# dbdexter-dev/meteor_demod

Measured on AMD Instinct MI355X. Metric: IQ Msamples/s demodulated (whole node), higher is better.
Workload: dtype f32

## Files before the change

meteor_demod_amd/csrc/demod_kernel_gat.hip:

```cpp
#include "rotwin_body.h"
#include "hip_host.h"

namespace {

typedef float gpair_t __attribute__((ext_vector_type(2)));
typedef float gquad_t __attribute__((ext_vector_type(4)));
typedef __attribute__((address_space(3))) const gquad_t lds_gquad;
typedef __attribute__((address_space(3))) const float lds_gfloat;

template <int FMT> struct GFmt;
template <> struct GFmt<16> {
	enum { G = 4 };
	__device__ static __forceinline__ gpair_t get(const uint4 &q, int k) { const uint32_t w = (&q.x)[k]; return gpair_t{ (float)(int)(int16_t)(w & 0xFFFFu), (float)((int)w >> 16) }; }
	__device__ static __forceinline__ gpair_t one(uint32_t w) { return gpair_t{ (float)(int)(int16_t)(w & 0xFFFFu), (float)((int)w >> 16) }; }
};
template <> struct GFmt<8> {
	enum { G = 8 };
	__device__ static __forceinline__ gpair_t get(const uint4 &q, int k) { const uint32_t w = (&q.x)[k >> 1] >> (16 * (k & 1)); return gpair_t{ (float)((int)(w & 0xFFu) - 128), (float)((int)((w >> 8) & 0xFFu) - 128) }; }
	__device__ static __forceinline__ gpair_t one(uint16_t w) { return gpair_t{ (float)((int)(w & 0xFFu) - 128), (float)((int)(w >> 8) - 128) }; }
};
template <> struct GFmt<32> {
	enum { G = 2 };
	__device__ static __forceinline__ gpair_t get(const uint4 &q, int k) { return gpair_t{ __uint_as_float((&q.x)[2 * k]), __uint_as_float((&q.x)[2 * k + 1]) }; }
	__device__ static __forceinline__ gpair_t one(float2 w) { return gpair_t{ w.x, w.y }; }
};

template <int KT, int FMT>
struct WinG {
	static constexpr int G = GFmt<FMT>::G, kTaps = KT, kBack = KT - 1, AMAX = G - 1, NS = KT + AMAX, NW = 4 * ((NS + 3) / 4), SLIDE = 4, MAXSL = 1, DEPTH = 1,
	                     BLOCK = MDEMOD_RW_BLOCK, ROTN = 1, RING = 32, REGSLOTS = 0;
	static constexpr bool GATHER = true;
	static_assert(NS % G == 0 && NS / G <= 36, "whole 16-byte loads, and few enough of them to stay in registers");
	typedef typename RFmt<FMT>::sample_t sample_t;
	__device__ __forceinline__ void setup(uint32_t) {}
	__device__ static __forceinline__ void put_history(const float2 *, bool, int) {}
	__device__ static __forceinline__ void put_init(const RGran<FMT> (&)[1], int) {}
	__device__ static __forceinline__ void put(const RGran<FMT> (&)[1], int) {}
	__device__ static __forceinline__ void fir(uint32_t, int, int, const DemodConsts &, int, float &, float &) {}

	__device__ static __forceinline__ void
	fir_gather(uint32_t ctab_addr, const sample_t *src, const float2 *hist, int v, int n, int bank, const DemodConsts &C, float &re, float &im)
	{
		const int oldest = v - kBack - (KT - 1);
		const int d = oldest & (G - 1);
		const int start = oldest - d;
		const int o = AMAX - d;
		const uint32_t row = ctab_addr + 4u * (uint32_t)(__mul24(bank * 4 + (o & 3), C.ctab_row_stride) + (o & ~3));
		gpair_t acc = { 0.0f, 0.0f };
		if (__builtin_expect(md_all(start >= 0 && start + NS <= n), 1)) {
			uint4 raw[NS / G];
#pragma unroll
			for (int g = 0; g < NS / G; g++) __builtin_memcpy(&raw[g], src + start + G * g, 16);
#pragma unroll
			for (int s4 = 0; s4 < NS / 4; s4++) {
				gquad_t c = { 0.0f, 0.0f, 0.0f, 0.0f };
				c = *(lds_gquad *)(row + 16u * (uint32_t)s4);
				const float cf[4] = { c.x, c.y, c.z, c.w };
#pragma unroll
				for (int k = 0; k < 4; k++) {
					const int slot = 4 * s4 + k;
					const gpair_t smp = GFmt<FMT>::get(raw[slot / G], slot % G);
					const gpair_t p = smp * cf[k];
					acc = acc + p;
				}
			}
			if constexpr (NS % 4 != 0) {
#pragma unroll
				for (int slot = NS / 4 * 4; slot < NS; slot++) {
					const float cf = *(lds_gfloat *)(row + 4u * (uint32_t)slot);
					const gpair_t p = GFmt<FMT>::get(raw[slot / G], slot % G) * cf;
					acc = acc + p;
				}
			}
		} else {
#pragma unroll 1
			for (int k = 0; k < KT; k++) {
				const int idx = oldest + k;
				gpair_t smp;
				if (idx < 0) { const float2 h = hist[kBack + idx]; smp.x = h.x; smp.y = h.y; }
				else smp = GFmt<FMT>::one(src[idx]);
				const float cf = *(lds_gfloat *)(row + 4u * (uint32_t)(d + k));
				const gpair_t p = smp * cf;
				acc = acc + p;
			}
		}
		re = acc.x; im = acc.y;
	}
};

template <int FMT, int OQPSK, int KT>
__global__ void __launch_bounds__(MDEMOD_RW_BLOCK, 2)
demod_kernel_gat(const DemodLaunch L)
{
	rotwin_demod<WinG<KT, FMT>, FMT, OQPSK, 0>(L);
}

template <int FMT, int OQPSK, int KT>
hipError_t
launch_gat(const DemodLaunch &L, size_t lds_bytes, hipStream_t stream)
{
	const uint32_t blocks = (L.n_streams + MDEMOD_RW_BLOCK - 1) / MDEMOD_RW_BLOCK;
	auto kfn = demod_kernel_gat<FMT, OQPSK, KT>;
	return mdm_launch(kfn, dim3(blocks), dim3(MDEMOD_RW_BLOCK), lds_bytes, stream, L);
}

}

template <int FMT>
static hipError_t
launch_gat_fmt(const DemodLaunch &L, int long_filter, size_t lds_bytes, hipStream_t stream)
{
	if constexpr (FMT != 32)
		if (long_filter) return L.c.oqpsk ? launch_gat<FMT, 1, 129>(L, lds_bytes, stream) : launch_gat<FMT, 0, 129>(L, lds_bytes, stream);
	if (long_filter) return hipErrorInvalidValue;
	return L.c.oqpsk ? launch_gat<FMT, 1, 65>(L, lds_bytes, stream) : launch_gat<FMT, 0, 65>(L, lds_bytes, stream);
}

hipError_t
mdemod_launch_demod_gat(const DemodLaunch &L, int fmt, int long_filter, size_t lds_bytes, hipStream_t stream)
{
	switch (fmt) {
	case 16: return launch_gat_fmt<16>(L, long_filter, lds_bytes, stream);
	case 8:  return launch_gat_fmt<8>(L, long_filter, lds_bytes, stream);
	case 32: return launch_gat_fmt<32>(L, long_filter, lds_bytes, stream);
	default: return hipErrorInvalidValue;
	}
}
```

meteor_demod_amd/csrc/demod_kernel_rot.hip:

```cpp
#include "rotwin_body.h"
#include "hip_host.h"
#ifdef ROTWIN_ASM_HEADER
#include ROTWIN_ASM_HEADER
#else
#include "rotwin_asm.h"
#endif

namespace {

static_assert(ROTWIN_NCH * 8 == 80, "window = ten chunks of eight");


__device__ __forceinline__ void
rot_fir(uint32_t row_addr, int rot, int flags, float &re, float &im)
{
	int tmp;
#if ROTWIN_PK == 1 || ROTWIN_PK == 3
	typedef float pair_t __attribute__((ext_vector_type(2)));
	pair_t acc = { 0.0f, 0.0f }, p0, p1;
	asm volatile(ROTWIN_FIR_ASM
	             : [acc] "+v"(acc), [p0] "=&v"(p0), [p1] "=&v"(p1), [tmp] "=&s"(tmp)
	             : [addr] "v"(row_addr), [rot] "s"(rot), [flags] "s"(flags)
	             : "vcc", "scc", ROTWIN_COEF_CLOBBERS);
	re = acc.x; im = acc.y;
#else
	float t0, t1, t2, t3;
	asm volatile(ROTWIN_FIR_ASM
	             : [ar] "=&v"(re), [ai] "=&v"(im), [t0] "=&v"(t0), [t1] "=&v"(t1), [t2] "=&v"(t2), [t3] "=&v"(t3), [tmp] "=&s"(tmp)
	             : [addr] "v"(row_addr), [rot] "s"(rot), [flags] "s"(flags)
	             : "vcc", "scc", ROTWIN_COEF_CLOBBERS);
#endif
}

template <int FMT> __device__ __forceinline__ void rot_put(const RGran<FMT> &a, const RGran<FMT> &b, int q);
template <> __device__ __forceinline__ void
rot_put<16>(const RGran<16> &a, const RGran<16> &b, int q)
{
	int tmp;
	asm volatile(ROTWIN_PUT_S16_ASM
	             : [tmp] "=&s"(tmp)
	             : [g0] "v"(a.w[0]), [g1] "v"(a.w[1]), [g2] "v"(a.w[2]), [g3] "v"(a.w[3]),
	               [g4] "v"(b.w[0]), [g5] "v"(b.w[1]), [g6] "v"(b.w[2]), [g7] "v"(b.w[3]), [rot] "s"(q)
	             : "vcc", "scc", "v255", "memory");
}
template <> __device__ __forceinline__ void
rot_put<8>(const RGran<8> &a, const RGran<8> &b, int q)
{
	const uint32_t g0 = a.w[0] ^ 0x80808080u, g1 = a.w[1] ^ 0x80808080u, g2 = b.w[0] ^ 0x80808080u, g3 = b.w[1] ^ 0x80808080u;
	int tmp;
	asm volatile(ROTWIN_PUT_U8_ASM
	             : [tmp] "=&s"(tmp)
	             : [g0] "v"(g0), [g1] "v"(g1), [g2] "v"(g2), [g3] "v"(g3), [rot] "s"(q)
	             : "vcc", "scc", "v255", "memory");
}
__device__ __forceinline__ void
rot_put_floats(const uint32_t (&f)[16], int q)
{
	int tmp;
	asm volatile(ROTWIN_PUT_F32_ASM
	             : [tmp] "=&s"(tmp)
	             : [f0] "v"(f[0]), [f1] "v"(f[1]), [f2] "v"(f[2]), [f3] "v"(f[3]), [f4] "v"(f[4]), [f5] "v"(f[5]), [f6] "v"(f[6]), [f7] "v"(f[7]),
	               [f8] "v"(f[8]), [f9] "v"(f[9]), [f10] "v"(f[10]), [f11] "v"(f[11]), [f12] "v"(f[12]), [f13] "v"(f[13]), [f14] "v"(f[14]), [f15] "v"(f[15]),
	               [rot] "s"(q)
	             : "vcc", "scc", "v255", "memory");
}
template <> __device__ __forceinline__ void
rot_put<32>(const RGran<32> &a, const RGran<32> &b, int q)
{
	uint32_t f[16];
#pragma unroll
	for (int i = 0; i < 8; i++) { f[i] = a.w[i]; f[8 + i] = b.w[i]; }
	rot_put_floats(f, q);
}

template <int FMT, int COMPACT = 0, int BLK = MDEMOD_RW_BLOCK>
struct WinF {
	static constexpr int kTaps = 65, kBack = 64, NW = 80, SLIDE = 8, AMAX = NW - kTaps, MAXSL = 1, DEPTH = 1, BLOCK = BLK, ROTN = NW / SLIDE, RING = 32;
	static constexpr bool GATHER = false;
	__device__ __forceinline__ void setup(uint32_t) {}
#ifndef ROT_REGSLOTS
#define ROT_REGSLOTS 0
#endif
	static constexpr int REGSLOTS = ROT_REGSLOTS;
	__device__ static __forceinline__ void put_history(const float2 *hist, bool valid, int q)
	{
		const uint4 *h4 = reinterpret_cast<const uint4 *>(hist);
		uint32_t f[16];
#pragma unroll
		for (int i = 0; i < 4; i++) {
			uint4 h = h4[i];
			if (!valid) h = make_uint4(0, 0, 0, 0);
			f[4 * i] = h.x; f[4 * i + 1] = h.y; f[4 * i + 2] = h.z; f[4 * i + 3] = h.w;
		}
		rot_put_floats(f, q);
	}
	__device__ static __forceinline__ void put(const RGran<FMT> (&g)[2], int q) { rot_put<FMT>(g[0], g[1], q); }
	__device__ static __forceinline__ void put_init(const RGran<FMT> (&g)[2], int q) { put(g, q); }
	__device__ static __forceinline__ void fir(uint32_t ctab_addr, int a, int bank, const DemodConsts &C, int rot, float &re, float &im)
	{
		const int o = AMAX - a;
		uint32_t row_addr;
		if (COMPACT) row_addr = rot_mad24((uint32_t)(bank * 4 + (o & 3)), 4u * (uint32_t)C.ctab_row_stride, ctab_addr + 4u * (uint32_t)(o & ~3));
		else row_addr = rot_mad24(rot_mad24((uint32_t)a, (uint32_t)C.interp, (uint32_t)bank), 4u * (uint32_t)C.ctab_row_stride, ctab_addr);
		static_assert(AMAX == 15, "two bits of a / 4");
		const int lo1 = md_all(a >= 8) ? 2 : 0, hi1 = md_all(a < 8) ? 1 : 3;
		const int q_lo = md_all(a >= 4 * (lo1 + 1)) ? lo1 + 1 : lo1, q_hi = md_all(a < 4 * hi1) ? hi1 - 1 : hi1;
		const int flags = ((1 << q_lo) - 1) | (((1 << (3 - q_hi)) - 1) << 3);
#ifdef ROT_EXP_NOSKIP
		int f0 = __builtin_amdgcn_readfirstlane(flags);
		asm volatile("s_and_b32 %0, %0, 0" : "+s"(f0) : : "scc");
		rot_fir(row_addr, rot, f0, re, im);
#else
		rot_fir(row_addr, rot, __builtin_amdgcn_readfirstlane(flags), re, im);
#endif
	}
};

typedef float pair_t2 __attribute__((ext_vector_type(2)));

template <int NA>
__device__ __forceinline__ void
rot_fir_acc(uint32_t addr, int rot, int last, pair_t2 &acc)
{
	int tmp;
	if constexpr (NA == 10)
		asm volatile(ROTWIN_FIR_ACC_ASM
		             : [acc] "+v"(acc), [tmp] "=&s"(tmp)
		             : [addr] "v"(addr), [rot] "s"(rot), [last] "s"(last)
		             : "vcc", "scc", ROTWIN_COEF_CLOBBERS, ROTWIN_ACC_CLOBBERS);
	else if constexpr (NA == 2)
		asm volatile(ROTWIN_FIR_ACC2_ASM
		             : [acc] "+v"(acc), [tmp] "=&s"(tmp)
		             : [addr] "v"(addr), [rot] "s"(rot), [last] "s"(last)
		             : "vcc", "scc", ROTWIN_COEF_CLOBBERS, ROTWIN_ACC_CLOBBERS);
	else
		asm volatile(ROTWIN_FIR_ACC5_ASM
		             : [acc] "+v"(acc), [tmp] "=&s"(tmp)
		             : [addr] "v"(addr), [rot] "s"(rot), [last] "s"(last)
		             : "vcc", "scc", ROTWIN_COEF_CLOBBERS, ROTWIN_ACC_CLOBBERS);
}
#define ROT_F16_OPERANDS \
	[f0] "v"(f[0]), [f1] "v"(f[1]), [f2] "v"(f[2]), [f3] "v"(f[3]), [f4] "v"(f[4]), [f5] "v"(f[5]), [f6] "v"(f[6]), [f7] "v"(f[7]), \
	[f8] "v"(f[8]), [f9] "v"(f[9]), [f10] "v"(f[10]), [f11] "v"(f[11]), [f12] "v"(f[12]), [f13] "v"(f[13]), [f14] "v"(f[14]), [f15] "v"(f[15])
template <int NA>
__device__ __forceinline__ void
rot_migrate(const uint32_t (&f)[16], int q)
{
	int tmp;
	if constexpr (NA == 10)
		asm volatile(ROTWIN_MIGRATE_ASM : [tmp] "=&s"(tmp) : ROT_F16_OPERANDS, [rot] "s"(q) : "vcc", "scc", "v255", ROTWIN_ACC_CLOBBERS, "memory");
	else if constexpr (NA == 2)
		asm volatile(ROTWIN_MIGRATE2_ASM : [tmp] "=&s"(tmp) : ROT_F16_OPERANDS, [rot] "s"(q) : "vcc", "scc", "v255", ROTWIN_ACC_CLOBBERS, "memory");
	else
		asm volatile(ROTWIN_MIGRATE5_ASM : [tmp] "=&s"(tmp) : ROT_F16_OPERANDS, [rot] "s"(q) : "vcc", "scc", "v255", ROTWIN_ACC_CLOBBERS, "memory");
}
template <int NA>
__device__ __forceinline__ void
rot_put_acc(const uint32_t (&f)[16], int q)
{
	int tmp;
	if constexpr (NA == 10)
		asm volatile(ROTWIN_PUT_ACC_ASM : [tmp] "=&s"(tmp) : ROT_F16_OPERANDS, [rot] "s"(q) : "vcc", "scc", ROTWIN_ACC_CLOBBERS, "memory");
	else if constexpr (NA == 2)
		asm volatile(ROTWIN_PUT_ACC2_ASM : [tmp] "=&s"(tmp) : ROT_F16_OPERANDS, [rot] "s"(q) : "vcc", "scc", ROTWIN_ACC_CLOBBERS, "memory");
	else
		asm volatile(ROTWIN_PUT_ACC5_ASM : [tmp] "=&s"(tmp) : ROT_F16_OPERANDS, [rot] "s"(q) : "vcc", "scc", ROTWIN_ACC_CLOBBERS, "memory");
}

template <int BLK, int NA, int MSL>
struct WinH {
	static constexpr int NR = 10, SLIDE = 8, NW = SLIDE * (NR + NA), kTaps = NA == 10 ? 129 : 65, kBack = kTaps - 1, AMAX = NW - kTaps, MAXSL = MSL, DEPTH = MSL,
	                     BLOCK = BLK, ROTN = NR, RING = 32, REGSLOTS = 0;
	static constexpr bool GATHER = false;
	static_assert((NA == 10 || NA == 2 || NA == 5) && AMAX == (NA == 5 ? 55 : 31) && kBack % SLIDE == 0, "wide (160 slots, 129 taps), mid (96 slots, 65 taps) or far (120 slots, 65 taps)");
	__device__ __forceinline__ void setup(uint32_t) {}
	__device__ static __forceinline__ void place(const uint32_t (&f)[16], int c)
	{
		if (c < NR) rot_put_floats(f, c);
		else rot_put_acc<NA>(f, c - NR);
	}
	__device__ static __forceinline__ void put_history(const float2 *hist, bool valid, int c)
	{
		const uint4 *h4 = reinterpret_cast<const uint4 *>(hist);
		uint32_t f[16];
#pragma unroll
		for (int i = 0; i < 4; i++) {
			uint4 h = h4[i];
			if (!valid) h = make_uint4(0, 0, 0, 0);
			f[4 * i] = h.x; f[4 * i + 1] = h.y; f[4 * i + 2] = h.z; f[4 * i + 3] = h.w;
		}
		place(f, c);
	}
	__device__ static __forceinline__ void put_init(const RGran<32> (&g)[2], int c)
	{
		uint32_t f[16];
#pragma unroll
		for (int i = 0; i < 8; i++) { f[i] = g[0].w[i]; f[8 + i] = g[1].w[i]; }
		place(f, c);
	}
	__device__ static __forceinline__ void put(const RGran<32> (&g)[2], int q)
	{
		uint32_t f[16];
#pragma unroll
		for (int i = 0; i < 8; i++) { f[i] = g[0].w[i]; f[8 + i] = g[1].w[i]; }
		rot_migrate<NA>(f, q);
	}
	__device__ static __forceinline__ void fir(uint32_t ctab_addr, int a, int bank, const DemodConsts &C, int rot, float &re, float &im)
	{
		const int o = AMAX - a;
		const uint32_t row = ctab_addr + 4u * (uint32_t)(__mul24(bank * 4 + (o & 3), C.ctab_row_stride) + (o & ~3));
		const int flags = (md_all(a >= 8) ? 3 : 0) | ((NA != 10 && md_all(a <= 7)) ? 16 : 0);
		rot_fir(row, rot, __builtin_amdgcn_readfirstlane(flags), re, im);
		if (NA == 10 || md_any(a >= 16)) {
			int last;
			if (NA == 10) last = 6 + (md_any(a >= 8) ? 1 : 0) + (md_any(a >= 16) ? 1 : 0) + (md_any(a >= 24) ? 1 : 0);
			else {
				last = md_any(a >= 24) ? 1 : 0;
				if (NA == 5) last += (md_any(a >= 32) ? 1 : 0) + (md_any(a >= 40) ? 1 : 0) + (md_any(a >= 48) ? 1 : 0);
			}
			pair_t2 acc = { re, im };
			rot_fir_acc<NA>(row + 4u * 80u, NA == 10 ? rot : (NA == 2 ? (rot & 1) : (rot >= 5 ? rot - 5 : rot)), __builtin_amdgcn_readfirstlane(last), acc);
			re = acc.x; im = acc.y;
		}
	}
};

template <int OQPSK, int BLK, int NA, int MSL>
__global__ void __launch_bounds__(BLK, 1) __attribute__((amdgpu_num_vgpr(ROTWIN_LIMIT)))
demod_kernel_roth(const DemodLaunch L)
{
	rotwin_demod<WinH<BLK, NA, MSL>, 32, OQPSK, 0>(L);
}

template <int FMT, int OQPSK, int KS, int COMPACT, int LUT>
__global__ void __launch_bounds__(LUT ? MDEMOD_RW_LUT_BLOCK : MDEMOD_RW_BLOCK, 2) __attribute__((amdgpu_num_vgpr(ROTWIN_LIMIT / 2)))
demod_kernel_rot(const DemodLaunch L)
{
	rotwin_demod<WinF<FMT, COMPACT, LUT ? MDEMOD_RW_LUT_BLOCK : MDEMOD_RW_BLOCK>, FMT, OQPSK, KS, LUT>(L);
}

template <int FMT, int OQPSK, int KS, int COMPACT = 0, int LUT = 0>
hipError_t
launch_rot_ks(const DemodLaunch &L, size_t lds_bytes, hipStream_t stream)
{
	constexpr int BLOCK = LUT ? MDEMOD_RW_LUT_BLOCK : MDEMOD_RW_BLOCK;
	const uint32_t blocks = (L.n_streams + BLOCK - 1) / BLOCK;
	auto kfn = demod_kernel_rot<FMT, OQPSK, KS, COMPACT, LUT>;
	return mdm_launch(kfn, dim3(blocks), dim3(BLOCK), lds_bytes, stream, L);
}

template <int FMT, int OQPSK>
hipError_t
launch_rot(const DemodLaunch &L, int compact, size_t lds_bytes, hipStream_t stream)
{
	constexpr int KS = OQPSK ? 6 : 14;
	if (compact) return launch_rot_ks<FMT, OQPSK, 0, 1>(L, lds_bytes, stream);
	return L.c.sin_lut && L.c.step_safe == KS && L.c.clock_tab ? launch_rot_ks<FMT, OQPSK, KS, 0, 1>(L, lds_bytes, stream) : launch_rot_ks<FMT, OQPSK, 0>(L, lds_bytes, stream);
}

}

template <int OQPSK, int BLK, int NA, int MSL>
static hipError_t
launch_roth(const DemodLaunch &L, size_t lds_bytes, hipStream_t stream)
{
	const uint32_t blocks = (L.n_streams + BLK - 1) / BLK;
	auto kfn = demod_kernel_roth<OQPSK, BLK, NA, MSL>;
	return mdm_launch(kfn, dim3(blocks), dim3(BLK), lds_bytes, stream, L);
}

hipError_t
mdemod_launch_demod_roth(const DemodLaunch &L, int geom, int many_slides, size_t lds_bytes, hipStream_t stream)
{
	if (geom == 1 && many_slides) return L.c.oqpsk ? launch_roth<1, 256, 2, 3>(L, lds_bytes, stream) : launch_roth<0, 256, 2, 3>(L, lds_bytes, stream);
	if (geom == 1) return L.c.oqpsk ? launch_roth<1, 256, 2, 2>(L, lds_bytes, stream) : launch_roth<0, 256, 2, 2>(L, lds_bytes, stream);
	if (geom == 2) return L.c.oqpsk ? launch_roth<1, 256, 5, 3>(L, lds_bytes, stream) : launch_roth<0, 256, 5, 3>(L, lds_bytes, stream);
	return L.c.oqpsk ? launch_roth<1, 256, 10, 2>(L, lds_bytes, stream) : launch_roth<0, 256, 10, 2>(L, lds_bytes, stream);
}

hipError_t
mdemod_launch_demod_rot(const DemodLaunch &L, int fmt, int compact, size_t lds_bytes, hipStream_t stream)
{
	switch (fmt) {
	case 16: return L.c.oqpsk ? launch_rot<16, 1>(L, compact, lds_bytes, stream) : launch_rot<16, 0>(L, compact, lds_bytes, stream);
	case 8:  return L.c.oqpsk ? launch_rot<8, 1>(L, compact, lds_bytes, stream) : launch_rot<8, 0>(L, compact, lds_bytes, stream);
	case 32: return L.c.oqpsk ? launch_rot<32, 1>(L, compact, lds_bytes, stream) : launch_rot<32, 0>(L, compact, lds_bytes, stream);
	default: return hipErrorInvalidValue;
	}
}
```

meteor_demod_amd/csrc/demod_kernel_rotp.hip:

```cpp
#include "rotwin_body.h"
#include "hip_host.h"
#ifdef ROTPK_ASM_HEADER
#include ROTPK_ASM_HEADER
#else
#include "rotpk_asm.h"
#endif

namespace {

typedef float pair_t __attribute__((ext_vector_type(2)));

template <int GEO> struct GeoP;
#ifndef ROTP_WIDE_DEPTH
#define ROTP_WIDE_DEPTH 1
#endif
#ifndef ROTP_MID_DEPTH
#define ROTP_MID_DEPTH 1
#endif
#ifndef ROTP_FAR_DEPTH
#define ROTP_FAR_DEPTH 2
#endif
template <> struct GeoP<0> { static constexpr int kTaps = 129, NW = MDEMOD_RW_WIDE_NW, MAXSL = 1, DEPTH = ROTP_WIDE_DEPTH, BLOCK = MDEMOD_RW_WIDE_BLOCK; };
template <> struct GeoP<1> { static constexpr int kTaps = 65, NW = MDEMOD_RW_MID_NW, MAXSL = 1, DEPTH = ROTP_MID_DEPTH, BLOCK = MDEMOD_RW_BLOCK; };
#ifndef ROTP_FAR_MAXSL
#define ROTP_FAR_MAXSL 2
#endif
template <> struct GeoP<2> { static constexpr int kTaps = 65, NW = MDEMOD_RW_FAR_NW, MAXSL = ROTP_FAR_MAXSL, DEPTH = ROTP_FAR_DEPTH, BLOCK = MDEMOD_RW_BLOCK; };
static_assert(MDEMOD_RW_WIDE_NW == 160 && MDEMOD_RW_MID_NW == 96 && MDEMOD_RW_FAR_NW == 112, "gen_rotpk_asm.py: GEOS");

template <int GEO, int FMT> struct AsmP;
#if ROTPK_FORM == 0
#define ROTP_FIR_CALL(TEXT, CLOB)                                                                                             \
	float ar = 0.0f, ai = 0.0f;                                                                                               \
	asm volatile(TEXT : [ar] "+v"(ar), [ai] "+v"(ai), [addr] "+v"(addr), [cnt] "+s"(cnt), [tmp] "=&s"(tmp)                    \
	             : [entry] "s"(entry), [sub] "s"(sub) : "vcc", "scc", CLOB);                                                \
	re = ar; im = ai;
#else
#define ROTP_FIR_CALL(TEXT, CLOB)                                                                                             \
	pair_t acc = { 0.0f, 0.0f };                                                                                              \
	asm volatile(TEXT : [acc] "+v"(acc), [addr] "+v"(addr), [cnt] "+s"(cnt), [tmp] "=&s"(tmp)                                 \
	             : [entry] "s"(entry), [sub] "s"(sub) : "vcc", "scc", CLOB);                                                \
	re = acc.x; im = acc.y;
#endif
#define ROTP_ASM(GEO, NAME, FMT)                                                                                              \
	template <> struct AsmP<GEO, FMT> {                                                                                       \
		__device__ static __forceinline__ void fir(uint32_t addr, int entry, int sub, int cnt, float &re, float &im)          \
		{                                                                                                                     \
			int tmp;                                                                                                          \
			ROTP_FIR_CALL(ROTPK_##NAME##_##FMT##_FIR_ASM, ROTPK_##NAME##_##FMT##_CLOBBERS)                                     \
		}                                                                                                                     \
		__device__ static __forceinline__ void put(const uint32_t (&g)[FMT == 16 ? 16 : 8], int q);                           \
	};
ROTP_ASM(0, WIDE, 16) ROTP_ASM(0, WIDE, 8) ROTP_ASM(1, MID, 16) ROTP_ASM(1, MID, 8) ROTP_ASM(2, FAR, 16) ROTP_ASM(2, FAR, 8)

#define ROTP_PUT16(GEO, NAME)                                                                                                 \
	__device__ __forceinline__ void AsmP<GEO, 16>::put(const uint32_t (&g)[16], int q)                                        \
	{                                                                                                                         \
		int tmp;                                                                                                              \
		asm volatile(ROTPK_##NAME##_16_PUT_ASM                                                                                \
		             : [tmp] "=&s"(tmp)                                                                                       \
		             : [g0] "v"(g[0]), [g1] "v"(g[1]), [g2] "v"(g[2]), [g3] "v"(g[3]), [g4] "v"(g[4]), [g5] "v"(g[5]), [g6] "v"(g[6]),  \
		               [g7] "v"(g[7]), [g8] "v"(g[8]), [g9] "v"(g[9]), [g10] "v"(g[10]), [g11] "v"(g[11]), [g12] "v"(g[12]),  \
		               [g13] "v"(g[13]), [g14] "v"(g[14]), [g15] "v"(g[15]), [rot] "s"(q)                                     \
		             : "vcc", "scc", "v255", "memory");                                                                       \
	}
#define ROTP_PUT8(GEO, NAME)                                                                                                  \
	__device__ __forceinline__ void AsmP<GEO, 8>::put(const uint32_t (&g)[8], int q)                                          \
	{                                                                                                                         \
		int tmp;                                                                                                              \
		asm volatile(ROTPK_##NAME##_8_PUT_ASM                                                                                 \
		             : [tmp] "=&s"(tmp)                                                                                       \
		             : [g0] "v"(g[0]), [g1] "v"(g[1]), [g2] "v"(g[2]), [g3] "v"(g[3]), [g4] "v"(g[4]), [g5] "v"(g[5]), [g6] "v"(g[6]),  \
		               [g7] "v"(g[7]), [rot] "s"(q)                                                                           \
		             : "vcc", "scc", "v255", "memory");                                                                       \
	}
ROTP_PUT16(0, WIDE) ROTP_PUT16(1, MID) ROTP_PUT16(2, FAR) ROTP_PUT8(0, WIDE) ROTP_PUT8(1, MID) ROTP_PUT8(2, FAR)

template <int GEO, int FMT>
struct WinP {
	static constexpr int kTaps = GeoP<GEO>::kTaps, kBack = kTaps - 1, NW = GeoP<GEO>::NW, SLIDE = 16, AMAX = NW - kTaps,
	                     MAXSL = GeoP<GEO>::MAXSL, DEPTH = GeoP<GEO>::DEPTH, BLOCK = GeoP<GEO>::BLOCK, NCH = NW / SLIDE, GD = FMT == 16 ? 16 : 8, REGSLOTS = 0, ROTN = NCH, RING = 32;
	static constexpr bool GATHER = false;
	__device__ __forceinline__ void setup(uint32_t) {}
	static_assert(kBack % SLIDE == 0 && NW % SLIDE == 0, "history and window are whole chunks");

	__device__ static __forceinline__ void put_history(const float2 *hist, bool valid, int q)
	{
		uint32_t g[GD];
#pragma unroll
		for (int k = 0; k < 16; k++) {
			float2 h = hist[k];
			if (!valid) h = make_float2(0.0f, 0.0f);
			if (FMT == 16) {
				g[k] = ((uint32_t)(int)h.x & 0xFFFFu) | ((uint32_t)(int)h.y << 16);
			} else {
				const uint32_t s = (uint32_t)(((int)h.x + 128) & 0xFF) | ((uint32_t)(((int)h.y + 128) & 0xFF) << 8);
				if (k & 1) g[k / 2] |= s << 16; else g[k / 2] = s;
			}
		}
		AsmP<GEO, FMT>::put(g, q);
	}
	__device__ static __forceinline__ void put(const RGran<FMT> (&gr)[4], int q)
	{
		uint32_t g[GD];
#pragma unroll
		for (int i = 0; i < 4; i++)
#pragma unroll
			for (int j = 0; j < GD / 4; j++) g[i * (GD / 4) + j] = gr[i].w[j];
		AsmP<GEO, FMT>::put(g, q);
	}
	__device__ static __forceinline__ void put_init(const RGran<FMT> (&gr)[4], int q) { put(gr, q); }
	__device__ static __forceinline__ void fir(uint32_t ctab_addr, int a, int bank, const DemodConsts &C, int rot, float &re, float &im)
	{
		const int o = AMAX - a;
		uint32_t addr = rot_mad24((uint32_t)(bank * 4 + (o & 3)), 4u * (uint32_t)C.ctab_row_stride, ctab_addr + 4u * (uint32_t)(o & ~3));
		constexpr int QB = AMAX / 4 >= 8 ? 4 : 3;
		static_assert(AMAX / 4 < (1 << QB) && (kTaps - 1) % 4 == 0, "alignments in groups of four");
		int q_lo = 0, q_hi = (1 << QB) - 1;
#pragma unroll
		for (int b = QB - 1; b >= 0; b--) {
			const int t = q_lo + (1 << b);
			q_lo = md_all(a >= 4 * t) ? t : q_lo;
			const int u = q_hi - (1 << b);
			q_hi = md_all(a < 4 * (u + 1)) ? u : q_hi;
		}
		q_lo = __builtin_amdgcn_readfirstlane(q_lo); q_hi = __builtin_amdgcn_readfirstlane(q_hi);
		const int c_lo = q_lo >> 2;
		int chunk = rot + c_lo;
		chunk = chunk >= NCH ? chunk - NCH : chunk;
		const int sub = q_lo & 3;
		constexpr int XS = ROTPK_EXIT / 4;
		const int cnt = (q_hi + (kTaps - 1) / 4) / XS - q_lo / XS;
		AsmP<GEO, FMT>::fir(addr + 64u * (uint32_t)c_lo, __builtin_amdgcn_readfirstlane(chunk), __builtin_amdgcn_readfirstlane(sub), __builtin_amdgcn_readfirstlane(cnt), re, im);
	}
};

#define ROTP_KERNEL(GEO, NAME, FMT, OQ)                                                                                       \
	__global__ void __launch_bounds__(GeoP<GEO>::BLOCK, 2) __attribute__((amdgpu_num_vgpr(ROTPK_##NAME##_##FMT##_LIMIT / 2)))  \
	demod_kernel_rotp_##NAME##_##FMT##_##OQ(const DemodLaunch L) { rotwin_demod<WinP<GEO, FMT>, FMT, OQ, 0>(L); }
__global__ void __launch_bounds__(GeoP<0>::BLOCK, 2) __attribute__((amdgpu_num_vgpr(ROTPK_WIDE_16_LIMIT / 2)))
demod_kernel_rotp_WIDE_16_0_ks109(const DemodLaunch L) { rotwin_demod<WinP<0, 16>, 16, 0, 109, 1>(L); }
ROTP_KERNEL(0, WIDE, 16, 0) ROTP_KERNEL(0, WIDE, 16, 1) ROTP_KERNEL(0, WIDE, 8, 0) ROTP_KERNEL(0, WIDE, 8, 1)
ROTP_KERNEL(1, MID, 16, 0) ROTP_KERNEL(1, MID, 16, 1) ROTP_KERNEL(1, MID, 8, 0) ROTP_KERNEL(1, MID, 8, 1)
ROTP_KERNEL(2, FAR, 16, 0) ROTP_KERNEL(2, FAR, 16, 1) ROTP_KERNEL(2, FAR, 8, 0) ROTP_KERNEL(2, FAR, 8, 1)

typedef void (*rotp_kernel_t)(const DemodLaunch);

hipError_t
launch_rotp(rotp_kernel_t kfn, int block, const DemodLaunch &L, size_t lds_bytes, hipStream_t stream)
{
	const uint32_t blocks = (L.n_streams + block - 1) / block;
	return mdm_launch(kfn, dim3(blocks), dim3(block), lds_bytes, stream, L);
}

}

hipError_t
mdemod_launch_demod_rotp(const DemodLaunch &L, int fmt, int geom , size_t lds_bytes, hipStream_t stream)
{
	if ((fmt != 16 && fmt != 8) || geom < 0 || geom > 2) return hipErrorInvalidValue;
	static const rotp_kernel_t table[3][2][2] = {
		{ { demod_kernel_rotp_WIDE_16_0, demod_kernel_rotp_WIDE_16_1 }, { demod_kernel_rotp_WIDE_8_0, demod_kernel_rotp_WIDE_8_1 } },
		{ { demod_kernel_rotp_MID_16_0, demod_kernel_rotp_MID_16_1 }, { demod_kernel_rotp_MID_8_0, demod_kernel_rotp_MID_8_1 } },
		{ { demod_kernel_rotp_FAR_16_0, demod_kernel_rotp_FAR_16_1 }, { demod_kernel_rotp_FAR_8_0, demod_kernel_rotp_FAR_8_1 } },
	};
	static const int blocks[3] = { GeoP<0>::BLOCK, GeoP<1>::BLOCK, GeoP<2>::BLOCK };
	if (geom == 0 && fmt == 16 && !L.c.oqpsk && L.c.step_safe == 109 && L.c.sin_lut) return launch_rotp(demod_kernel_rotp_WIDE_16_0_ks109, blocks[0], L, lds_bytes, stream);
	return launch_rotp(table[geom][fmt == 16 ? 0 : 1][L.c.oqpsk ? 1 : 0], blocks[geom], L, lds_bytes, stream);
}
```

meteor_demod_amd/csrc/gen_rotwin_asm.py:

```python
#!/usr/bin/env python3
import os
import sys

WB = 96
CB = None
NCH = 10
PAIRWAIT = int(os.environ.get("ROTWIN_PAIRWAIT", "1"))
DC = int(os.environ.get("ROTWIN_DC", "1"))
NBUF = 2 * (DC + 1) if PAIRWAIT else 4
CB = 96 - 4 * NBUF
PK = int(os.environ.get("ROTWIN_PK", "1"))
TB = CB - 4
CHB = 32


def q(lines):
    return "\n".join('\t"%s\\n\\t"' % l for l in lines)


def jump(tag, n):
    return [
        "s_getpc_b64 vcc",
        ".L%s_pc_%%=:" % tag,
        "s_mul_i32 %%[tmp], %%[rot], (.L%s_1_%%= - .L%s_0_%%=)" % (tag, tag),
        "s_add_u32 %%[tmp], %%[tmp], (.L%s_0_%%= - .L%s_pc_%%=)" % (tag, tag),
        "s_add_u32 vcc_lo, vcc_lo, %[tmp]",
        "s_addc_u32 vcc_hi, vcc_hi, 0",
        "s_setpc_b64 vcc",
    ]


def fir():
    NH, D = 2 * NCH, 3
    def load(h):
        b = CB + 4 * (h % NBUF)
        return "ds_read_b128 v[%d:%d], %%[addr] offset:%d" % (b, b + 3, 16 * h)
    L = []
    if PK in (0, 2):
        L += ["v_mov_b32 %[ar], 0", "v_mov_b32 %[ai], 0"]
    L += [load(h) for h in range(2 * DC if PAIRWAIT else D)]
    L += jump("fir", NCH)
    for r in range(NCH):
        L += [".Lfir_%d_%%=:" % r]
        for h in range(NH):
            c = h // 2
            if PAIRWAIT:
                if h % 2 == 0:
                    L += [load(x) for x in (h + 2 * DC, h + 2 * DC + 1) if x < NH]
                    L += ["s_waitcnt lgkmcnt(%d)" % min(2 * DC, max(0, NH - 2 - h))]
            else:
                if h + D < NH:
                    L += [load(h + D)]
                L += ["s_waitcnt lgkmcnt(%d)" % min(D, NH - 1 - h)]
            if h < 3:
                L += ["s_bitcmp1_b32 %%[flags], %d" % h, "s_cbranch_scc1 .Lfir_%d_s%d_%%=" % (r, h)]
            if h >= NH - 3:
                L += ["s_bitcmp1_b32 %%[flags], %d" % (3 + NH - 1 - h), "s_cbranch_scc1 .Lfir_%d_s9_%%=" % r]
            hb = CB + 4 * (h % NBUF)
            wq = WB + 16 * ((c + r) % NCH) + 8 * (h & 1)
            if PK == 1:
                def mul(j):
                    return ["v_pk_mul_f32 %%[p%d], v[%d:%d], v[%d:%d] op_sel:[0,%d] op_sel_hi:[1,%d]"
                            % (j & 1, wq + 2 * j, wq + 2 * j + 1, hb + 2 * (j // 2), hb + 2 * (j // 2) + 1, j & 1, j & 1)]
                def add(j):
                    return ["v_pk_add_f32 %%[acc], %%[acc], %%[p%d]" % (j & 1)]
            elif PK == 2:
                def mul(j):
                    t = TB + 2 * (j & 1)
                    return ["v_pk_mul_f32 v[%d:%d], v[%d:%d], v[%d:%d] op_sel:[0,%d] op_sel_hi:[1,%d]"
                            % (t, t + 1, wq + 2 * j, wq + 2 * j + 1, hb + 2 * (j // 2), hb + 2 * (j // 2) + 1, j & 1, j & 1)]
                def add(j):
                    t = TB + 2 * (j & 1)
                    return ["v_add_f32 %%[ar], %%[ar], v%d" % t, "v_add_f32 %%[ai], %%[ai], v%d" % (t + 1)]
            elif PK == 3:
                def mul(j):
                    t = TB + 2 * (j & 1)
                    return ["v_mul_f32 v%d, v%d, v%d" % (t, hb + j, wq + 2 * j), "v_mul_f32 v%d, v%d, v%d" % (t + 1, hb + j, wq + 2 * j + 1)]
                def add(j):
                    t = TB + 2 * (j & 1)
                    return ["v_pk_add_f32 %%[acc], %%[acc], v[%d:%d]" % (t, t + 1)]
            else:
                def mul(j):
                    t = "%%[t%d]" % (2 * (j & 1)), "%%[t%d]" % (2 * (j & 1) + 1)
                    return ["v_mul_f32 %s, v%d, v%d" % (t[0], hb + j, wq + 2 * j),
                            "v_mul_f32 %s, v%d, v%d" % (t[1], hb + j, wq + 2 * j + 1)]
                def add(j):
                    t = "%%[t%d]" % (2 * (j & 1)), "%%[t%d]" % (2 * (j & 1) + 1)
                    return ["v_add_f32 %%[ar], %%[ar], %s" % t[0], "v_add_f32 %%[ai], %%[ai], %s" % t[1]]
            L += mul(0)
            for j in range(4):
                if j + 1 < 4:
                    L += mul(j + 1)
                L += add(j)
            if h < 3:
                L += [".Lfir_%d_s%d_%%=:" % (r, h)]
        L += [".Lfir_%d_s9_%%=:" % r, "s_branch .Lfir_end_%="]
    L += [".Lfir_end_%=:", "s_waitcnt lgkmcnt(0)"]
    return L


def put(kind):
    L = ["s_nop 1"] if kind == "u8" else []
    L += jump("put", NCH)
    for r in range(NCH):
        L += [".Lput_%d_%%=:" % r]
        wq = WB + 16 * r
        for s in range(8):
            for comp in range(2):
                dst = wq + 2 * s + comp
                if kind == "s16":
                    L += ["v_cvt_f32_i32_sdwa v%d, sext(%%[g%d]) dst_sel:DWORD dst_unused:UNUSED_PAD src0_sel:WORD_%d" % (dst, s, comp)]
                elif kind == "u8":
                    L += ["v_cvt_f32_i32_sdwa v%d, sext(%%[g%d]) dst_sel:DWORD dst_unused:UNUSED_PAD src0_sel:BYTE_%d" % (dst, s // 2, 2 * (s & 1) + comp)]
                else:
                    L += ["v_mov_b32 v%d, %%[f%d]" % (dst, 2 * s + comp)]
        L += ["s_branch .Lput_end_%="]
    L += [".Lput_end_%=:"]
    return L


AB = 96


def fir_acc(NA, tag):
    NH = 2 * NA
    lo = 6 if NA == NCH else 0
    def load(h):
        b = CB + 4 * (h % 3)
        return "ds_read_b128 v[%d:%d], %%[addr] offset:%d" % (b, b + 3, 16 * h)
    L = [load(h) for h in range(2)]
    L += jump(tag, NA)
    for r in range(NA):
        L += [".L%s_%d_%%=:" % (tag, r)]
        for h in range(NH):
            c = h // 2
            if h + 2 < NH:
                L += [load(h + 2)]
            L += ["s_waitcnt lgkmcnt(%d)" % min(2, NH - 1 - h)]
            hb = CB + 4 * (h % 3)
            aq = AB + 16 * ((c + r) % NA) + 8 * (h & 1)
            def rd(j):
                t = CB + 12 + 2 * (j & 1)
                return ["v_accvgpr_read_b32 v%d, a%d" % (t, aq + 2 * j), "v_accvgpr_read_b32 v%d, a%d" % (t + 1, aq + 2 * j + 1)]
            def mul(j):
                t = CB + 12 + 2 * (j & 1)
                return ["v_pk_mul_f32 v[%d:%d], v[%d:%d], v[%d:%d] op_sel:[0,%d] op_sel_hi:[1,%d]" % (t, t + 1, t, t + 1, hb + 2 * (j // 2), hb + 2 * (j // 2) + 1, j & 1, j & 1)]
            def add(j):
                t = CB + 12 + 2 * (j & 1)
                return ["v_pk_add_f32 %%[acc], %%[acc], v[%d:%d]" % (t, t + 1)]
            L += rd(0) + rd(1) + mul(0) + mul(1) + add(0) + rd(2) + add(1) + rd(3) + mul(2) + mul(3) + add(2) + add(3)
            if h % 2 == 1 and lo <= c < NA - 1:
                L += ["s_cmp_eq_u32 %%[last], %d" % c, "s_cbranch_scc1 .L%s_end_%%=" % tag]
        L += ["s_branch .L%s_end_%%=" % tag]
    L += [".L%s_end_%%=:" % tag, "s_waitcnt lgkmcnt(0)"]
    return L


def migrate(NA, tag):
    assert NCH % NA == 0
    L = jump(tag, NCH)
    for r in range(NCH):
        L += [".L%s_%d_%%=:" % (tag, r)]
        L += ["v_accvgpr_read_b32 v%d, a%d" % (WB + 16 * r + k, AB + 16 * (r % NA) + k) for k in range(16)]
        L += ["v_accvgpr_write_b32 a%d, %%[f%d]" % (AB + 16 * (r % NA) + k, k) for k in range(16)]
        L += ["s_branch .L%s_end_%%=" % tag]
    L += [".L%s_end_%%=:" % tag]
    return L


def put_acc(NA, tag):
    L = jump(tag, NA)
    for r in range(NA):
        L += [".L%s_%d_%%=:" % (tag, r)]
        L += ["v_accvgpr_write_b32 a%d, %%[f%d]" % (AB + 16 * r + k, k) for k in range(16)]
        L += ["s_branch .L%s_end_%%=" % tag]
    L += [".L%s_end_%%=:" % tag]
    return L


def main():
    out = []
    out.append("/* GENERATED by gen_rotwin_asm.py - do not edit.  gfx950 assembly of the rotating register window. */")
    out.append("#ifndef MDEMOD_ROTWIN_ASM_H")
    out.append("#define MDEMOD_ROTWIN_ASM_H")
    out.append("#define ROTWIN_WB %d" % WB)
    out.append("#define ROTWIN_CB %d" % CB)
    out.append("#define ROTWIN_LIMIT %d   /* first register the compiler may not use */" % (TB if PK in (2, 3) else CB))
    out.append("#define ROTWIN_NCH %d" % NCH)
    out.append("#define ROTWIN_AB %d   /* first AccVGPR of the hybrid window's newer half */" % AB)
    out.append("#define ROTWIN_PK %d" % PK)
    out.append("#define ROTWIN_FIR_ASM \\\n" + q(fir()).replace("\n", " \\\n"))
    for kind in ("s16", "u8", "f32"):
        out.append("#define ROTWIN_PUT_%s_ASM \\\n" % kind.upper() + q(put(kind)).replace("\n", " \\\n"))
    for NA, sfx in ((NCH, ""), (2, "2"), (5, "5")):
        out.append("#define ROTWIN_FIR_ACC%s_ASM \\\n" % sfx + q(fir_acc(NA, "fira" + sfx)).replace("\n", " \\\n"))
        out.append("#define ROTWIN_MIGRATE%s_ASM \\\n" % sfx + q(migrate(NA, "mig" + sfx)).replace("\n", " \\\n"))
        out.append("#define ROTWIN_PUT_ACC%s_ASM \\\n" % sfx + q(put_acc(NA, "puta" + sfx)).replace("\n", " \\\n"))
    out.append("#define ROTWIN_ACC_CLOBBERS " + ", ".join('"a%d"' % i for i in range(AB, AB + 16 * NCH)))
    out.append("#define ROTWIN_COEF_CLOBBERS " + ", ".join('"v%d"' % i for i in range(TB if PK in (2, 3) else CB, WB)))
    out.append("#endif")
    sys.stdout.write("\n".join(out) + "\n")


if __name__ == "__main__":
    main()
```

meteor_demod_amd/csrc/rotwin_asm.h:

```cpp
#ifndef MDEMOD_ROTWIN_ASM_H
#define MDEMOD_ROTWIN_ASM_H
#define ROTWIN_WB 96
#define ROTWIN_CB 80
#define ROTWIN_LIMIT 80
#define ROTWIN_NCH 10
#define ROTWIN_AB 96
#define ROTWIN_PK 1
#define ROTWIN_FIR_ASM \
	"ds_read_b128 v[80:83], %[addr] offset:0\n\t" \
	"ds_read_b128 v[84:87], %[addr] offset:16\n\t" \
	"s_getpc_b64 vcc\n\t" \
	".Lfir_pc_%=:\n\t" \
	"s_mul_i32 %[tmp], %[rot], (.Lfir_1_%= - .Lfir_0_%=)\n\t" \
	"s_add_u32 %[tmp], %[tmp], (.Lfir_0_%= - .Lfir_pc_%=)\n\t" \
	"s_add_u32 vcc_lo, vcc_lo, %[tmp]\n\t" \
	"s_addc_u32 vcc_hi, vcc_hi, 0\n\t" \
	"s_setpc_b64 vcc\n\t" \
	".Lfir_0_%=:\n\t" \
	"ds_read_b128 v[88:91], %[addr] offset:32\n\t" \
	"ds_read_b128 v[92:95], %[addr] offset:48\n\t" \
	"s_waitcnt lgkmcnt(2)\n\t" \
	"s_bitcmp1_b32 %[flags], 0\n\t" \
	"s_cbranch_scc1 .Lfir_0_s0_%=\n\t" \
	"v_pk_mul_f32 %[p0], v[96:97], v[80:81] op_sel:[0,0] op_sel_hi:[1,0]\n\t" \
	"v_pk_mul_f32 %[p1], v[98:99], v[80:81] op_sel:[0,1] op_sel_hi:[1,1]\n\t" \
	"v_pk_add_f32 %[acc], %[acc], %[p0]\n\t" \
	"v_pk_mul_f32 %[p0], v[100:101], v[82:83] op_sel:[0,0] op_sel_hi:[1,0]\n\t" \
	"v_pk_add_f32 %[acc], %[acc], %[p1]\n\t" \
	"v_pk_mul_f32 %[p1], v[102:103], v[82:83] op_sel:[0,1] op_sel_hi:[1,1]\n\t" \
	"v_pk_add_f32 %[acc], %[acc], %[p0]\n\t" \
	"v_pk_add_f32 %[acc], %[acc], %[p1]\n\t" \
	".Lfir_0_s0_%=:\n\t" \
	"s_bitcmp1_b32 %[flags], 1\n\t" \
	"s_cbranch_scc1 .Lfir_0_s1_%=\n\t" \
	"v_pk_mul_f32 %[p0], v[104:105], v[84:85] op_sel:[0,0] op_sel_hi:[1,0]\n\t" \
	"v_pk_mul_f32 %[p1], v[106:107], v[84:85] op_sel:[0,1] op_sel_hi:[1,1]\n\t" \
	"v_pk_add_f32 %[acc], %[acc], %[p0]\n\t" \
	"v_pk_mul_f32 %[p0], v[108:109], v[86:87] op_sel:[0,0] op_sel_hi:[1,0]\n\t" \
	"v_pk_add_f32 %[acc], %[acc], %[p1]\n\t" \
	"v_pk_mul_f32 %[p1], v[110:111], v[86:87] op_sel:[0,1] op_sel_hi:[1,1]\n\t" \
	"v_pk_add_f32 %[acc], %[acc], %[p0]\n\t" \
	"v_pk_add_f32 %[acc], %[acc], %[p1]\n\t" \
	".Lfir_0_s1_%=:\n\t" \
	"ds_read_b128 v[80:83], %[addr] offset:64\n\t" \
	"ds_read_b128 v[84:87], %[addr] offset:80\n\t" \
	"s_waitcnt lgkmcnt(2)\n\t" \
	"s_bitcmp1_b32 %[flags], 2\n\t" \
	"s_cbranch_scc1 .Lfir_0_s2_%=\n\t" \
	"v_pk_mul_f32 %[p0], v[112:113], v[88:89] op_sel:[0,0] op_sel_hi:[1,0]\n\t" \
	"v_pk_mul_f32 %[p1], v[114:115], v[88:89] op_sel:[0,1] op_sel_hi:[1,1]\n\t" \
	"v_pk_add_f32 %[acc], %[acc], %[p0]\n\t" \
	"v_pk_mul_f32 %[p0], v[116:117], v[90:91] op_sel:[0,0] op_sel_hi:[1,0]\n\t" \
	"v_pk_add_f32 %[acc], %[acc], %[p1]\n\t" \
	"v_pk_mul_f32 %[p1], v[118:119], v[90:91] op_sel:[0,1] op_sel_hi:[1,1]\n\t" \
	"v_pk_add_f32 %[acc], %[acc], %[p0]\n\t" \
	"v_pk_add_f32 %[acc], %[acc], %[p1]\n\t" \
	".Lfir_0_s2_%=:\n\t" \
	"v_pk_mul_f32 %[p0], v[120:121], v[92:93] op_sel:[0,0] op_sel_hi:[1,0]\n\t" \
	"v_pk_mul_f32 %[p1], v[122:123], v[92:93] op_sel:[0,1] op_sel_hi:[1,1]\n\t" \
	"v_pk_add_f32 %[acc], %[acc], %[p0]\n\t" \
	"v_pk_mul_f32 %[p0], v[124:125], v[94:95] op_sel:[0,0] op_sel_hi:[1,0]\n\t" \
	"v_pk_add_f32 %[acc], %[acc], %[p1]\n\t" \
	"v_pk_mul_f32 %[p1], v[126:127], v[94:95] op_sel:[0,1] op_sel_hi:[1,1]\n\t" \
	"v_pk_add_f32 %[acc], %[acc], %[p0]\n\t" \
	"v_pk_add_f32 %[acc], %[acc], %[p1]\n\t" \
	"ds_read_b128 v[88:91], %[addr] offset:96\n\t" \
	"ds_read_b128 v[92:95], %[addr] offset:112\n\t" \
	"s_waitcnt lgkmcnt(2)\n\t" \
	"v_pk_mul_f32 %[p0], v[128:129], v[80:81] op_sel:[0,0] op_sel_hi:[1,0]\n\t" \
	"v_pk_mul_f32 %[p1], v[130:131], v[80:81] op_sel:[0,1] op_sel_hi:[1,1]\n\t" \
	"v_pk_add_f32 %[acc], %[acc], %[p0]\n\t" \
	"v_pk_mul_f32 %[p0], v[132:133], v[82:83] op_sel:[0,0] op_sel_hi:[1,0]\n\t" \
	"v_pk_add_f32 %[acc], %[acc], %[p1]\n\t" \
	"v_pk_mul_f32 %[p1], v[134:135], v[82:83] op_sel:[0,1] op_sel_hi:[1,1]\n\t" \
	"v_pk_add_f32 %[acc], %[acc], %[p0]\n\t" \
	"v_pk_add_f32 %[acc], %[acc], %[p1]\n\t" \
	"v_pk_mul_f32 %[p0], v[136:137], v[84:85] op_sel:[0,0] op_sel_hi:[1,0]\n\t" \
	"v_pk_mul_f32 %[p1], v[138:139], v[84:85] op_sel:[0,1] op_sel_hi:[1,1]\n\t" \
	"v_pk_add_f32 %[acc], %[acc], %[p0]\n\t" \
	"v_pk_mul_f32 %[p0], v[140:141], v[86:87] op_sel:[0,0] op_sel_hi:[1,0]\n\t" \
	"v_pk_add_f32 %[acc], %[acc], %[p1]\n\t" \
	"v_pk_mul_f32 %[p1], v[142:143], v[86:87] op_sel:[0,1] op_sel_hi:[1,1]\n\t" \
	"v_pk_add_f32 %[acc], %[acc], %[p0]\n\t" \
	"v_pk_add_f32 %[acc], %[acc], %[p1]\n\t" \
	"ds_read_b128 v[80:83], %[addr] offset:128\n\t" \
	"ds_read_b128 v[84:87], %[addr] offset:144\n\t" \
	"s_waitcnt lgkmcnt(2)\n\t" \
	"v_pk_mul_f32 %[p0], v[144:145], v[88:89] op_sel:[0,0] op_sel_hi:[1,0]\n\t" \
	"v_pk_mul_f32 %[p1], v[146:147], v[88:89] op_sel:[0,1] op_sel_hi:[1,1]\n\t" \
	"v_pk_add_f32 %[acc], %[acc], %[p0]\n\t" \
	"v_pk_mul_f32 %[p0], v[148:149], v[90:91] op_sel:[0,0] op_sel_hi:[1,0]\n\t" \
	"v_pk_add_f32 %[acc], %[acc], %[p1]\n\t" \
	"v_pk_mul_f32 %[p1], v[150:151], v[90:91] op_sel:[0,1] op_sel_hi:[1,1]\n\t" \
	"v_pk_add_f32 %[acc], %[acc], %[p0]\n\t" \
	"v_pk_add_f32 %[acc], %[acc], %[p1]\n\t" \
	"v_pk_mul_f32 %[p0], v[152:153], v[92:93] op_sel:[0,0] op_sel_hi:[1,0]\n\t" \
	"v_pk_mul_f32 %[p1], v[154:155], v[92:93] op_sel:[0,1] op_sel_hi:[1,1]\n\t" \
	"v_pk_add_f32 %[acc], %[acc], %[p0]\n\t" \
	"v_pk_mul_f32 %[p0], v[156:157], v[94:95] op_sel:[0,0] op_sel_hi:[1,0]\n\t" \
	"v_pk_add_f32 %[acc], %[acc], %[p1]\n\t" \
	"v_pk_mul_f32 %[p1], v[158:159], v[94:95] op_sel:[0,1] op_sel_hi:[1,1]\n\t" \
	"v_pk_add_f32 %[acc], %[acc], %[p0]\n\t" \
	"v_pk_add_f32 %[acc], %[acc], %[p1]\n\t" \
	"ds_read_b128 v[88:91], %[addr] offset:160\n\t" \
	"ds_read_b128 v[92:95], %[addr] offset:176\n\t" \
	"s_waitcnt lgkmcnt(2)\n\t" \
	"v_pk_mul_f32 %[p0], v[160:161], v[80:81] op_sel:[0,0] op_sel_hi:[1,0]\n\t" \
	"v_pk_mul_f32 %[p1], v[162:163], v[80:81] op_sel:[0,1] op_sel_hi:[1,1]\n\t" \
	"v_pk_add_f32 %[acc], %[acc], %[p0]\n\t" \
	"v_pk_mul_f32 %[p0], v[164:165], v[82:83] op_sel:[0,0] op_sel_hi:[1,0]\n\t" \
	"v_pk_add_f32 %[acc], %[acc], %[p1]\n\t" \
	"v_pk_mul_f32 %[p1], v[166:167], v[82:83] op_sel:[0,1] op_sel_hi:[1,1]\n\t" \
	"v_pk_add_f32 %[acc], %[acc], %[p0]\n\t" \
	"v_pk_add_f32 %[acc], %[acc], %[p1]\n\t" \
	"v_pk_mul_f32 %[p0], v[168:169], v[84:85] op_sel:[0,0] op_sel_hi:[1,0]\n\t" \
	"v_pk_mul_f32 %[p1], v[170:171], v[84:85] op_sel:[0,1] op_sel_hi:[1,1]\n\t" \
	"v_pk_add_f32 %[acc], %[acc], %[p0]\n\t" \
	"v_pk_mul_f32 %[p0], v[172:173], v[86:87] op_sel:[0,0] op_sel_hi:[1,0]\n\t" \
	"v_pk_add_f32 %[acc], %[acc], %[p1]\n\t" \
	"v_pk_mul_f32 %[p1], v[174:175], v[86:87] op_sel:[0,1] op_sel_hi:[1,1]\n\t" \
	"v_pk_add_f32 %[acc], %[acc], %[p0]\n\t" \
	"v_pk_add_f32 %[acc], %[acc], %[p1]\n\t" \
	"ds_read_b128 v[80:83], %[addr] offset:192\n\t" \
	"ds_read_b128 v[84:87], %[addr] offset:208\n\t" \
	"s_waitcnt lgkmcnt(2)\n\t" \
	"v_pk_mul_f32 %[p0], v[176:177], v[88:89] op_sel:[0,0] op_sel_hi:[1,0]\n\t" \
	"v_pk_mul_f32 %[p1], v[178:179], v[88:89] op_sel:[0,1] op_sel_hi:[1,1]\n\t" \
	"v_pk_add_f32 %[acc], %[acc], %[p0]\n\t" \
	"v_pk_mul_f32 %[p0], v[180:181], v[90:91] op_sel:[0,0] op_sel_hi:[1,0]\n\t" \
	"v_pk_add_f32 %[acc], %[acc], %[p1]\n\t" \
	"v_pk_mul_f32 %[p1], v[182:183], v[90:91] op_sel:[0,1] op_sel_hi:[1,1]\n\t" \
	"v_pk_add_f32 %[acc], %[acc], %[p0]\n\t" \
	"v_pk_add_f32 %[acc], %[acc], %[p1]\n\t" \
	"v_pk_mul_f32 %[p0], v[184:185], v[92:93] op_sel:[0,0] op_sel_hi:[1,0]\n\t" \
	"v_pk_mul_f32 %[p1], v[186:187], v[92:93] op_sel:[0,1] op_sel_hi:[1,1]\n\t" \
	"v_pk_add_f32 %[acc], %[acc], %[p0]\n\t" \
	"v_pk_mul_f32 %[p0], v[188:189], v[94:95] op_sel:[0,0] op_sel_hi:[1,0]\n\t" \
	"v_pk_add_f32 %[acc], %[acc], %[p1]\n\t" \
	"v_pk_mul_f32 %[p1], v[190:191], v[94:95] op_sel:[0,1] op_sel_hi:[1,1]\n\t" \
	"v_pk_add_f32 %[acc], %[acc], %[p0]\n\t" \
	"v_pk_add_f32 %[acc], %[acc], %[p1]\n\t" \
	"ds_read_b128 v[88:91], %[addr] offset:224\n\t" \
	"ds_read_b128 v[92:95], %[addr] offset:240\n\t" \
	"s_waitcnt lgkmcnt(2)\n\t" \
	"v_pk_mul_f32 %[p0], v[192:193], v[80:81] op_sel:[0,0] op_sel_hi:[1,0]\n\t" \
	"v_pk_mul_f32 %[p1], v[194:195], v[80:81] op_sel:[0,1] op_sel_hi:[1,1]\n\t" \
	"v_pk_add_f32 %[acc], %[acc], %[p0]\n\t" \
	"v_pk_mul_f32 %[p0], v[196:197], v[82:83] op_sel:[0,0] op_sel_hi:[1,0]\n\t" \
	"v_pk_add_f32 %[acc], %[acc], %[p1]\n\t" \
	"v_pk_mul_f32 %[p1], v[198:199], v[82:83] op_sel:[0,1] op_sel_hi:[1,1]\n\t" \
	"v_pk_add_f32 %[acc], %[acc], %[p0]\n\t" \
	"v_pk_add_f32 %[acc], %[acc], %[p1]\n\t" \
	"v_pk_mul_f32 %[p0], v[200:201], v[84:85] op_sel:[0,0] op_sel_hi:[1,0]\n\t" \
	"v_pk_mul_f32 %[p1], v[202:203], v[84:85] op_sel:[0,1] op_sel_hi:[1,1]\n\t" \
	"v_pk_add_f32 %[acc], %[acc], %[p0]\n\t" \
	"v_pk_mul_f32 %[p0], v[204:205], v[86:87] op_sel:[0,0] op_sel_hi:[1,0]\n\t" \
	"v_pk_add_f32 %[acc], %[acc], %[p1]\n\t" \
	"v_pk_mul_f32 %[p1], v[206:207], v[86:87] op_sel:[0,1] op_sel_hi:[1,1]\n\t" \
	"v_pk_add_f32 %[acc], %[acc], %[p0]\n\t" \
	"v_pk_add_f32 %[acc], %[acc], %[p1]\n\t" \
	"ds_read_b128 v[80:83], %[addr] offset:256\n\t" \
// ... 1953 lines not shown
	"v_cvt_f32_i32_sdwa v120, sext(%[g4]) dst_sel:DWORD dst_unused:UNUSED_PAD src0_sel:WORD_0\n\t" \
	"v_cvt_f32_i32_sdwa v121, sext(%[g4]) dst_sel:DWORD dst_unused:UNUSED_PAD src0_sel:WORD_1\n\t" \
	"v_cvt_f32_i32_sdwa v122, sext(%[g5]) dst_sel:DWORD dst_unused:UNUSED_PAD src0_sel:WORD_0\n\t" \
	"v_cvt_f32_i32_sdwa v123, sext(%[g5]) dst_sel:DWORD dst_unused:UNUSED_PAD src0_sel:WORD_1\n\t" \
	"v_cvt_f32_i32_sdwa v124, sext(%[g6]) dst_sel:DWORD dst_unused:UNUSED_PAD src0_sel:WORD_0\n\t" \
	"v_cvt_f32_i32_sdwa v125, sext(%[g6]) dst_sel:DWORD dst_unused:UNUSED_PAD src0_sel:WORD_1\n\t" \
	"v_cvt_f32_i32_sdwa v126, sext(%[g7]) dst_sel:DWORD dst_unused:UNUSED_PAD src0_sel:WORD_0\n\t" \
	"v_cvt_f32_i32_sdwa v127, sext(%[g7]) dst_sel:DWORD dst_unused:UNUSED_PAD src0_sel:WORD_1\n\t" \
	"s_branch .Lput_end_%=\n\t" \
	".Lput_2_%=:\n\t" \
	"v_cvt_f32_i32_sdwa v128, sext(%[g0]) dst_sel:DWORD dst_unused:UNUSED_PAD src0_sel:WORD_0\n\t" \
	"v_cvt_f32_i32_sdwa v129, sext(%[g0]) dst_sel:DWORD dst_unused:UNUSED_PAD src0_sel:WORD_1\n\t" \
	"v_cvt_f32_i32_sdwa v130, sext(%[g1]) dst_sel:DWORD dst_unused:UNUSED_PAD src0_sel:WORD_0\n\t" \
	"v_cvt_f32_i32_sdwa v131, sext(%[g1]) dst_sel:DWORD dst_unused:UNUSED_PAD src0_sel:WORD_1\n\t" \
	"v_cvt_f32_i32_sdwa v132, sext(%[g2]) dst_sel:DWORD dst_unused:UNUSED_PAD src0_sel:WORD_0\n\t" \
	"v_cvt_f32_i32_sdwa v133, sext(%[g2]) dst_sel:DWORD dst_unused:UNUSED_PAD src0_sel:WORD_1\n\t" \
	"v_cvt_f32_i32_sdwa v134, sext(%[g3]) dst_sel:DWORD dst_unused:UNUSED_PAD src0_sel:WORD_0\n\t" \
	"v_cvt_f32_i32_sdwa v135, sext(%[g3]) dst_sel:DWORD dst_unused:UNUSED_PAD src0_sel:WORD_1\n\t" \
	"v_cvt_f32_i32_sdwa v136, sext(%[g4]) dst_sel:DWORD dst_unused:UNUSED_PAD src0_sel:WORD_0\n\t" \
	"v_cvt_f32_i32_sdwa v137, sext(%[g4]) dst_sel:DWORD dst_unused:UNUSED_PAD src0_sel:WORD_1\n\t" \
	"v_cvt_f32_i32_sdwa v138, sext(%[g5]) dst_sel:DWORD dst_unused:UNUSED_PAD src0_sel:WORD_0\n\t" \
	"v_cvt_f32_i32_sdwa v139, sext(%[g5]) dst_sel:DWORD dst_unused:UNUSED_PAD src0_sel:WORD_1\n\t" \
	"v_cvt_f32_i32_sdwa v140, sext(%[g6]) dst_sel:DWORD dst_unused:UNUSED_PAD src0_sel:WORD_0\n\t" \
	"v_cvt_f32_i32_sdwa v141, sext(%[g6]) dst_sel:DWORD dst_unused:UNUSED_PAD src0_sel:WORD_1\n\t" \
	"v_cvt_f32_i32_sdwa v142, sext(%[g7]) dst_sel:DWORD dst_unused:UNUSED_PAD src0_sel:WORD_0\n\t" \
	"v_cvt_f32_i32_sdwa v143, sext(%[g7]) dst_sel:DWORD dst_unused:UNUSED_PAD src0_sel:WORD_1\n\t" \
	"s_branch .Lput_end_%=\n\t" \
	".Lput_3_%=:\n\t" \
	"v_cvt_f32_i32_sdwa v144, sext(%[g0]) dst_sel:DWORD dst_unused:UNUSED_PAD src0_sel:WORD_0\n\t" \
	"v_cvt_f32_i32_sdwa v145, sext(%[g0]) dst_sel:DWORD dst_unused:UNUSED_PAD src0_sel:WORD_1\n\t" \
	"v_cvt_f32_i32_sdwa v146, sext(%[g1]) dst_sel:DWORD dst_unused:UNUSED_PAD src0_sel:WORD_0\n\t" \
	"v_cvt_f32_i32_sdwa v147, sext(%[g1]) dst_sel:DWORD dst_unused:UNUSED_PAD src0_sel:WORD_1\n\t" \
	"v_cvt_f32_i32_sdwa v148, sext(%[g2]) dst_sel:DWORD dst_unused:UNUSED_PAD src0_sel:WORD_0\n\t" \
	"v_cvt_f32_i32_sdwa v149, sext(%[g2]) dst_sel:DWORD dst_unused:UNUSED_PAD src0_sel:WORD_1\n\t" \
	"v_cvt_f32_i32_sdwa v150, sext(%[g3]) dst_sel:DWORD dst_unused:UNUSED_PAD src0_sel:WORD_0\n\t" \
	"v_cvt_f32_i32_sdwa v151, sext(%[g3]) dst_sel:DWORD dst_unused:UNUSED_PAD src0_sel:WORD_1\n\t" \
	"v_cvt_f32_i32_sdwa v152, sext(%[g4]) dst_sel:DWORD dst_unused:UNUSED_PAD src0_sel:WORD_0\n\t" \
	"v_cvt_f32_i32_sdwa v153, sext(%[g4]) dst_sel:DWORD dst_unused:UNUSED_PAD src0_sel:WORD_1\n\t" \
	"v_cvt_f32_i32_sdwa v154, sext(%[g5]) dst_sel:DWORD dst_unused:UNUSED_PAD src0_sel:WORD_0\n\t" \
	"v_cvt_f32_i32_sdwa v155, sext(%[g5]) dst_sel:DWORD dst_unused:UNUSED_PAD src0_sel:WORD_1\n\t" \
	"v_cvt_f32_i32_sdwa v156, sext(%[g6]) dst_sel:DWORD dst_unused:UNUSED_PAD src0_sel:WORD_0\n\t" \
	"v_cvt_f32_i32_sdwa v157, sext(%[g6]) dst_sel:DWORD dst_unused:UNUSED_PAD src0_sel:WORD_1\n\t" \
	"v_cvt_f32_i32_sdwa v158, sext(%[g7]) dst_sel:DWORD dst_unused:UNUSED_PAD src0_sel:WORD_0\n\t" \
	"v_cvt_f32_i32_sdwa v159, sext(%[g7]) dst_sel:DWORD dst_unused:UNUSED_PAD src0_sel:WORD_1\n\t" \
	"s_branch .Lput_end_%=\n\t" \
	".Lput_4_%=:\n\t" \
	"v_cvt_f32_i32_sdwa v160, sext(%[g0]) dst_sel:DWORD dst_unused:UNUSED_PAD src0_sel:WORD_0\n\t" \
	"v_cvt_f32_i32_sdwa v161, sext(%[g0]) dst_sel:DWORD dst_unused:UNUSED_PAD src0_sel:WORD_1\n\t" \
	"v_cvt_f32_i32_sdwa v162, sext(%[g1]) dst_sel:DWORD dst_unused:UNUSED_PAD src0_sel:WORD_0\n\t" \
	"v_cvt_f32_i32_sdwa v163, sext(%[g1]) dst_sel:DWORD dst_unused:UNUSED_PAD src0_sel:WORD_1\n\t" \
	"v_cvt_f32_i32_sdwa v164, sext(%[g2]) dst_sel:DWORD dst_unused:UNUSED_PAD src0_sel:WORD_0\n\t" \
	"v_cvt_f32_i32_sdwa v165, sext(%[g2]) dst_sel:DWORD dst_unused:UNUSED_PAD src0_sel:WORD_1\n\t" \
	"v_cvt_f32_i32_sdwa v166, sext(%[g3]) dst_sel:DWORD dst_unused:UNUSED_PAD src0_sel:WORD_0\n\t" \
	"v_cvt_f32_i32_sdwa v167, sext(%[g3]) dst_sel:DWORD dst_unused:UNUSED_PAD src0_sel:WORD_1\n\t" \
	"v_cvt_f32_i32_sdwa v168, sext(%[g4]) dst_sel:DWORD dst_unused:UNUSED_PAD src0_sel:WORD_0\n\t" \
	"v_cvt_f32_i32_sdwa v169, sext(%[g4]) dst_sel:DWORD dst_unused:UNUSED_PAD src0_sel:WORD_1\n\t" \
	"v_cvt_f32_i32_sdwa v170, sext(%[g5]) dst_sel:DWORD dst_unused:UNUSED_PAD src0_sel:WORD_0\n\t" \
	"v_cvt_f32_i32_sdwa v171, sext(%[g5]) dst_sel:DWORD dst_unused:UNUSED_PAD src0_sel:WORD_1\n\t" \
	"v_cvt_f32_i32_sdwa v172, sext(%[g6]) dst_sel:DWORD dst_unused:UNUSED_PAD src0_sel:WORD_0\n\t" \
	"v_cvt_f32_i32_sdwa v173, sext(%[g6]) dst_sel:DWORD dst_unused:UNUSED_PAD src0_sel:WORD_1\n\t" \
	"v_cvt_f32_i32_sdwa v174, sext(%[g7]) dst_sel:DWORD dst_unused:UNUSED_PAD src0_sel:WORD_0\n\t" \
	"v_cvt_f32_i32_sdwa v175, sext(%[g7]) dst_sel:DWORD dst_unused:UNUSED_PAD src0_sel:WORD_1\n\t" \
	"s_branch .Lput_end_%=\n\t" \
	".Lput_5_%=:\n\t" \
	"v_cvt_f32_i32_sdwa v176, sext(%[g0]) dst_sel:DWORD dst_unused:UNUSED_PAD src0_sel:WORD_0\n\t" \
	"v_cvt_f32_i32_sdwa v177, sext(%[g0]) dst_sel:DWORD dst_unused:UNUSED_PAD src0_sel:WORD_1\n\t" \
	"v_cvt_f32_i32_sdwa v178, sext(%[g1]) dst_sel:DWORD dst_unused:UNUSED_PAD src0_sel:WORD_0\n\t" \
	"v_cvt_f32_i32_sdwa v179, sext(%[g1]) dst_sel:DWORD dst_unused:UNUSED_PAD src0_sel:WORD_1\n\t" \
	"v_cvt_f32_i32_sdwa v180, sext(%[g2]) dst_sel:DWORD dst_unused:UNUSED_PAD src0_sel:WORD_0\n\t" \
	"v_cvt_f32_i32_sdwa v181, sext(%[g2]) dst_sel:DWORD dst_unused:UNUSED_PAD src0_sel:WORD_1\n\t" \
	"v_cvt_f32_i32_sdwa v182, sext(%[g3]) dst_sel:DWORD dst_unused:UNUSED_PAD src0_sel:WORD_0\n\t" \
	"v_cvt_f32_i32_sdwa v183, sext(%[g3]) dst_sel:DWORD dst_unused:UNUSED_PAD src0_sel:WORD_1\n\t" \
	"v_cvt_f32_i32_sdwa v184, sext(%[g4]) dst_sel:DWORD dst_unused:UNUSED_PAD src0_sel:WORD_0\n\t" \
	"v_cvt_f32_i32_sdwa v185, sext(%[g4]) dst_sel:DWORD dst_unused:UNUSED_PAD src0_sel:WORD_1\n\t" \
	"v_cvt_f32_i32_sdwa v186, sext(%[g5]) dst_sel:DWORD dst_unused:UNUSED_PAD src0_sel:WORD_0\n\t" \
	"v_cvt_f32_i32_sdwa v187, sext(%[g5]) dst_sel:DWORD dst_unused:UNUSED_PAD src0_sel:WORD_1\n\t" \
	"v_cvt_f32_i32_sdwa v188, sext(%[g6]) dst_sel:DWORD dst_unused:UNUSED_PAD src0_sel:WORD_0\n\t" \
	"v_cvt_f32_i32_sdwa v189, sext(%[g6]) dst_sel:DWORD dst_unused:UNUSED_PAD src0_sel:WORD_1\n\t" \
	"v_cvt_f32_i32_sdwa v190, sext(%[g7]) dst_sel:DWORD dst_unused:UNUSED_PAD src0_sel:WORD_0\n\t" \
	"v_cvt_f32_i32_sdwa v191, sext(%[g7]) dst_sel:DWORD dst_unused:UNUSED_PAD src0_sel:WORD_1\n\t" \
	"s_branch .Lput_end_%=\n\t" \
	".Lput_6_%=:\n\t" \
	"v_cvt_f32_i32_sdwa v192, sext(%[g0]) dst_sel:DWORD dst_unused:UNUSED_PAD src0_sel:WORD_0\n\t" \
	"v_cvt_f32_i32_sdwa v193, sext(%[g0]) dst_sel:DWORD dst_unused:UNUSED_PAD src0_sel:WORD_1\n\t" \
	"v_cvt_f32_i32_sdwa v194, sext(%[g1]) dst_sel:DWORD dst_unused:UNUSED_PAD src0_sel:WORD_0\n\t" \
	"v_cvt_f32_i32_sdwa v195, sext(%[g1]) dst_sel:DWORD dst_unused:UNUSED_PAD src0_sel:WORD_1\n\t" \
	"v_cvt_f32_i32_sdwa v196, sext(%[g2]) dst_sel:DWORD dst_unused:UNUSED_PAD src0_sel:WORD_0\n\t" \
	"v_cvt_f32_i32_sdwa v197, sext(%[g2]) dst_sel:DWORD dst_unused:UNUSED_PAD src0_sel:WORD_1\n\t" \
	"v_cvt_f32_i32_sdwa v198, sext(%[g3]) dst_sel:DWORD dst_unused:UNUSED_PAD src0_sel:WORD_0\n\t" \
	"v_cvt_f32_i32_sdwa v199, sext(%[g3]) dst_sel:DWORD dst_unused:UNUSED_PAD src0_sel:WORD_1\n\t" \
	"v_cvt_f32_i32_sdwa v200, sext(%[g4]) dst_sel:DWORD dst_unused:UNUSED_PAD src0_sel:WORD_0\n\t" \
	"v_cvt_f32_i32_sdwa v201, sext(%[g4]) dst_sel:DWORD dst_unused:UNUSED_PAD src0_sel:WORD_1\n\t" \
	"v_cvt_f32_i32_sdwa v202, sext(%[g5]) dst_sel:DWORD dst_unused:UNUSED_PAD src0_sel:WORD_0\n\t" \
	"v_cvt_f32_i32_sdwa v203, sext(%[g5]) dst_sel:DWORD dst_unused:UNUSED_PAD src0_sel:WORD_1\n\t" \
	"v_cvt_f32_i32_sdwa v204, sext(%[g6]) dst_sel:DWORD dst_unused:UNUSED_PAD src0_sel:WORD_0\n\t" \
	"v_cvt_f32_i32_sdwa v205, sext(%[g6]) dst_sel:DWORD dst_unused:UNUSED_PAD src0_sel:WORD_1\n\t" \
	"v_cvt_f32_i32_sdwa v206, sext(%[g7]) dst_sel:DWORD dst_unused:UNUSED_PAD src0_sel:WORD_0\n\t" \
	"v_cvt_f32_i32_sdwa v207, sext(%[g7]) dst_sel:DWORD dst_unused:UNUSED_PAD src0_sel:WORD_1\n\t" \
	"s_branch .Lput_end_%=\n\t" \
	".Lput_7_%=:\n\t" \
	"v_cvt_f32_i32_sdwa v208, sext(%[g0]) dst_sel:DWORD dst_unused:UNUSED_PAD src0_sel:WORD_0\n\t" \
	"v_cvt_f32_i32_sdwa v209, sext(%[g0]) dst_sel:DWORD dst_unused:UNUSED_PAD src0_sel:WORD_1\n\t" \
	"v_cvt_f32_i32_sdwa v210, sext(%[g1]) dst_sel:DWORD dst_unused:UNUSED_PAD src0_sel:WORD_0\n\t" \
	"v_cvt_f32_i32_sdwa v211, sext(%[g1]) dst_sel:DWORD dst_unused:UNUSED_PAD src0_sel:WORD_1\n\t" \
	"v_cvt_f32_i32_sdwa v212, sext(%[g2]) dst_sel:DWORD dst_unused:UNUSED_PAD src0_sel:WORD_0\n\t" \
	"v_cvt_f32_i32_sdwa v213, sext(%[g2]) dst_sel:DWORD dst_unused:UNUSED_PAD src0_sel:WORD_1\n\t" \
	"v_cvt_f32_i32_sdwa v214, sext(%[g3]) dst_sel:DWORD dst_unused:UNUSED_PAD src0_sel:WORD_0\n\t" \
	"v_cvt_f32_i32_sdwa v215, sext(%[g3]) dst_sel:DWORD dst_unused:UNUSED_PAD src0_sel:WORD_1\n\t" \
	"v_cvt_f32_i32_sdwa v216, sext(%[g4]) dst_sel:DWORD dst_unused:UNUSED_PAD src0_sel:WORD_0\n\t" \
	"v_cvt_f32_i32_sdwa v217, sext(%[g4]) dst_sel:DWORD dst_unused:UNUSED_PAD src0_sel:WORD_1\n\t" \
	"v_cvt_f32_i32_sdwa v218, sext(%[g5]) dst_sel:DWORD dst_unused:UNUSED_PAD src0_sel:WORD_0\n\t" \
	"v_cvt_f32_i32_sdwa v219, sext(%[g5]) dst_sel:DWORD dst_unused:UNUSED_PAD src0_sel:WORD_1\n\t" \
	"v_cvt_f32_i32_sdwa v220, sext(%[g6]) dst_sel:DWORD dst_unused:UNUSED_PAD src0_sel:WORD_0\n\t" \
	"v_cvt_f32_i32_sdwa v221, sext(%[g6]) dst_sel:DWORD dst_unused:UNUSED_PAD src0_sel:WORD_1\n\t" \
	"v_cvt_f32_i32_sdwa v222, sext(%[g7]) dst_sel:DWORD dst_unused:UNUSED_PAD src0_sel:WORD_0\n\t" \
	"v_cvt_f32_i32_sdwa v223, sext(%[g7]) dst_sel:DWORD dst_unused:UNUSED_PAD src0_sel:WORD_1\n\t" \
	"s_branch .Lput_end_%=\n\t" \
	".Lput_8_%=:\n\t" \
	"v_cvt_f32_i32_sdwa v224, sext(%[g0]) dst_sel:DWORD dst_unused:UNUSED_PAD src0_sel:WORD_0\n\t" \
	"v_cvt_f32_i32_sdwa v225, sext(%[g0]) dst_sel:DWORD dst_unused:UNUSED_PAD src0_sel:WORD_1\n\t" \
	"v_cvt_f32_i32_sdwa v226, sext(%[g1]) dst_sel:DWORD dst_unused:UNUSED_PAD src0_sel:WORD_0\n\t" \
	"v_cvt_f32_i32_sdwa v227, sext(%[g1]) dst_sel:DWORD dst_unused:UNUSED_PAD src0_sel:WORD_1\n\t" \
	"v_cvt_f32_i32_sdwa v228, sext(%[g2]) dst_sel:DWORD dst_unused:UNUSED_PAD src0_sel:WORD_0\n\t" \
	"v_cvt_f32_i32_sdwa v229, sext(%[g2]) dst_sel:DWORD dst_unused:UNUSED_PAD src0_sel:WORD_1\n\t" \
	"v_cvt_f32_i32_sdwa v230, sext(%[g3]) dst_sel:DWORD dst_unused:UNUSED_PAD src0_sel:WORD_0\n\t" \
	"v_cvt_f32_i32_sdwa v231, sext(%[g3]) dst_sel:DWORD dst_unused:UNUSED_PAD src0_sel:WORD_1\n\t" \
	"v_cvt_f32_i32_sdwa v232, sext(%[g4]) dst_sel:DWORD dst_unused:UNUSED_PAD src0_sel:WORD_0\n\t" \
	"v_cvt_f32_i32_sdwa v233, sext(%[g4]) dst_sel:DWORD dst_unused:UNUSED_PAD src0_sel:WORD_1\n\t" \
	"v_cvt_f32_i32_sdwa v234, sext(%[g5]) dst_sel:DWORD dst_unused:UNUSED_PAD src0_sel:WORD_0\n\t" \
	"v_cvt_f32_i32_sdwa v235, sext(%[g5]) dst_sel:DWORD dst_unused:UNUSED_PAD src0_sel:WORD_1\n\t" \
	"v_cvt_f32_i32_sdwa v236, sext(%[g6]) dst_sel:DWORD dst_unused:UNUSED_PAD src0_sel:WORD_0\n\t" \
	"v_cvt_f32_i32_sdwa v237, sext(%[g6]) dst_sel:DWORD dst_unused:UNUSED_PAD src0_sel:WORD_1\n\t" \
	"v_cvt_f32_i32_sdwa v238, sext(%[g7]) dst_sel:DWORD dst_unused:UNUSED_PAD src0_sel:WORD_0\n\t" \
	"v_cvt_f32_i32_sdwa v239, sext(%[g7]) dst_sel:DWORD dst_unused:UNUSED_PAD src0_sel:WORD_1\n\t" \
	"s_branch .Lput_end_%=\n\t" \
	".Lput_9_%=:\n\t" \
	"v_cvt_f32_i32_sdwa v240, sext(%[g0]) dst_sel:DWORD dst_unused:UNUSED_PAD src0_sel:WORD_0\n\t" \
	"v_cvt_f32_i32_sdwa v241, sext(%[g0]) dst_sel:DWORD dst_unused:UNUSED_PAD src0_sel:WORD_1\n\t" \
	"v_cvt_f32_i32_sdwa v242, sext(%[g1]) dst_sel:DWORD dst_unused:UNUSED_PAD src0_sel:WORD_0\n\t" \
	"v_cvt_f32_i32_sdwa v243, sext(%[g1]) dst_sel:DWORD dst_unused:UNUSED_PAD src0_sel:WORD_1\n\t" \
	"v_cvt_f32_i32_sdwa v244, sext(%[g2]) dst_sel:DWORD dst_unused:UNUSED_PAD src0_sel:WORD_0\n\t" \
	"v_cvt_f32_i32_sdwa v245, sext(%[g2]) dst_sel:DWORD dst_unused:UNUSED_PAD src0_sel:WORD_1\n\t" \
	"v_cvt_f32_i32_sdwa v246, sext(%[g3]) dst_sel:DWORD dst_unused:UNUSED_PAD src0_sel:WORD_0\n\t" \
	"v_cvt_f32_i32_sdwa v247, sext(%[g3]) dst_sel:DWORD dst_unused:UNUSED_PAD src0_sel:WORD_1\n\t" \
	"v_cvt_f32_i32_sdwa v248, sext(%[g4]) dst_sel:DWORD dst_unused:UNUSED_PAD src0_sel:WORD_0\n\t" \
	"v_cvt_f32_i32_sdwa v249, sext(%[g4]) dst_sel:DWORD dst_unused:UNUSED_PAD src0_sel:WORD_1\n\t" \
	"v_cvt_f32_i32_sdwa v250, sext(%[g5]) dst_sel:DWORD dst_unused:UNUSED_PAD src0_sel:WORD_0\n\t" \
	"v_cvt_f32_i32_sdwa v251, sext(%[g5]) dst_sel:DWORD dst_unused:UNUSED_PAD src0_sel:WORD_1\n\t" \
	"v_cvt_f32_i32_sdwa v252, sext(%[g6]) dst_sel:DWORD dst_unused:UNUSED_PAD src0_sel:WORD_0\n\t" \
	"v_cvt_f32_i32_sdwa v253, sext(%[g6]) dst_sel:DWORD dst_unused:UNUSED_PAD src0_sel:WORD_1\n\t" \
	"v_cvt_f32_i32_sdwa v254, sext(%[g7]) dst_sel:DWORD dst_unused:UNUSED_PAD src0_sel:WORD_0\n\t" \
	"v_cvt_f32_i32_sdwa v255, sext(%[g7]) dst_sel:DWORD dst_unused:UNUSED_PAD src0_sel:WORD_1\n\t" \
	"s_branch .Lput_end_%=\n\t" \
	".Lput_end_%=:\n\t"
#define ROTWIN_PUT_U8_ASM \
	"s_nop 1\n\t" \
	"s_getpc_b64 vcc\n\t" \
	".Lput_pc_%=:\n\t" \
	"s_mul_i32 %[tmp], %[rot], (.Lput_1_%= - .Lput_0_%=)\n\t" \
	"s_add_u32 %[tmp], %[tmp], (.Lput_0_%= - .Lput_pc_%=)\n\t" \
	"s_add_u32 vcc_lo, vcc_lo, %[tmp]\n\t" \
	"s_addc_u32 vcc_hi, vcc_hi, 0\n\t" \
	"s_setpc_b64 vcc\n\t" \
	".Lput_0_%=:\n\t" \
	"v_cvt_f32_i32_sdwa v96, sext(%[g0]) dst_sel:DWORD dst_unused:UNUSED_PAD src0_sel:BYTE_0\n\t" \
	"v_cvt_f32_i32_sdwa v97, sext(%[g0]) dst_sel:DWORD dst_unused:UNUSED_PAD src0_sel:BYTE_1\n\t" \
	"v_cvt_f32_i32_sdwa v98, sext(%[g0]) dst_sel:DWORD dst_unused:UNUSED_PAD src0_sel:BYTE_2\n\t" \
	"v_cvt_f32_i32_sdwa v99, sext(%[g0]) dst_sel:DWORD dst_unused:UNUSED_PAD src0_sel:BYTE_3\n\t" \
	"v_cvt_f32_i32_sdwa v100, sext(%[g1]) dst_sel:DWORD dst_unused:UNUSED_PAD src0_sel:BYTE_0\n\t" \
	"v_cvt_f32_i32_sdwa v101, sext(%[g1]) dst_sel:DWORD dst_unused:UNUSED_PAD src0_sel:BYTE_1\n\t" \
	"v_cvt_f32_i32_sdwa v102, sext(%[g1]) dst_sel:DWORD dst_unused:UNUSED_PAD src0_sel:BYTE_2\n\t" \
	"v_cvt_f32_i32_sdwa v103, sext(%[g1]) dst_sel:DWORD dst_unused:UNUSED_PAD src0_sel:BYTE_3\n\t" \
	"v_cvt_f32_i32_sdwa v104, sext(%[g2]) dst_sel:DWORD dst_unused:UNUSED_PAD src0_sel:BYTE_0\n\t" \
	"v_cvt_f32_i32_sdwa v105, sext(%[g2]) dst_sel:DWORD dst_unused:UNUSED_PAD src0_sel:BYTE_1\n\t" \
	"v_cvt_f32_i32_sdwa v106, sext(%[g2]) dst_sel:DWORD dst_unused:UNUSED_PAD src0_sel:BYTE_2\n\t" \
	"v_cvt_f32_i32_sdwa v107, sext(%[g2]) dst_sel:DWORD dst_unused:UNUSED_PAD src0_sel:BYTE_3\n\t" \
	"v_cvt_f32_i32_sdwa v108, sext(%[g3]) dst_sel:DWORD dst_unused:UNUSED_PAD src0_sel:BYTE_0\n\t" \
	"v_cvt_f32_i32_sdwa v109, sext(%[g3]) dst_sel:DWORD dst_unused:UNUSED_PAD src0_sel:BYTE_1\n\t" \
	"v_cvt_f32_i32_sdwa v110, sext(%[g3]) dst_sel:DWORD dst_unused:UNUSED_PAD src0_sel:BYTE_2\n\t" \
	"v_cvt_f32_i32_sdwa v111, sext(%[g3]) dst_sel:DWORD dst_unused:UNUSED_PAD src0_sel:BYTE_3\n\t" \
	"s_branch .Lput_end_%=\n\t" \
	".Lput_1_%=:\n\t" \
	"v_cvt_f32_i32_sdwa v112, sext(%[g0]) dst_sel:DWORD dst_unused:UNUSED_PAD src0_sel:BYTE_0\n\t" \
	"v_cvt_f32_i32_sdwa v113, sext(%[g0]) dst_sel:DWORD dst_unused:UNUSED_PAD src0_sel:BYTE_1\n\t" \
	"v_cvt_f32_i32_sdwa v114, sext(%[g0]) dst_sel:DWORD dst_unused:UNUSED_PAD src0_sel:BYTE_2\n\t" \
	"v_cvt_f32_i32_sdwa v115, sext(%[g0]) dst_sel:DWORD dst_unused:UNUSED_PAD src0_sel:BYTE_3\n\t" \
	"v_cvt_f32_i32_sdwa v116, sext(%[g1]) dst_sel:DWORD dst_unused:UNUSED_PAD src0_sel:BYTE_0\n\t" \
	"v_cvt_f32_i32_sdwa v117, sext(%[g1]) dst_sel:DWORD dst_unused:UNUSED_PAD src0_sel:BYTE_1\n\t" \
	"v_cvt_f32_i32_sdwa v118, sext(%[g1]) dst_sel:DWORD dst_unused:UNUSED_PAD src0_sel:BYTE_2\n\t" \
	"v_cvt_f32_i32_sdwa v119, sext(%[g1]) dst_sel:DWORD dst_unused:UNUSED_PAD src0_sel:BYTE_3\n\t" \
	"v_cvt_f32_i32_sdwa v120, sext(%[g2]) dst_sel:DWORD dst_unused:UNUSED_PAD src0_sel:BYTE_0\n\t" \
	"v_cvt_f32_i32_sdwa v121, sext(%[g2]) dst_sel:DWORD dst_unused:UNUSED_PAD src0_sel:BYTE_1\n\t" \
	"v_cvt_f32_i32_sdwa v122, sext(%[g2]) dst_sel:DWORD dst_unused:UNUSED_PAD src0_sel:BYTE_2\n\t" \
	"v_cvt_f32_i32_sdwa v123, sext(%[g2]) dst_sel:DWORD dst_unused:UNUSED_PAD src0_sel:BYTE_3\n\t" \
	"v_cvt_f32_i32_sdwa v124, sext(%[g3]) dst_sel:DWORD dst_unused:UNUSED_PAD src0_sel:BYTE_0\n\t" \
	"v_cvt_f32_i32_sdwa v125, sext(%[g3]) dst_sel:DWORD dst_unused:UNUSED_PAD src0_sel:BYTE_1\n\t" \
	"v_cvt_f32_i32_sdwa v126, sext(%[g3]) dst_sel:DWORD dst_unused:UNUSED_PAD src0_sel:BYTE_2\n\t" \
	"v_cvt_f32_i32_sdwa v127, sext(%[g3]) dst_sel:DWORD dst_unused:UNUSED_PAD src0_sel:BYTE_3\n\t" \
	"s_branch .Lput_end_%=\n\t" \
	".Lput_2_%=:\n\t" \
	"v_cvt_f32_i32_sdwa v128, sext(%[g0]) dst_sel:DWORD dst_unused:UNUSED_PAD src0_sel:BYTE_0\n\t" \
	"v_cvt_f32_i32_sdwa v129, sext(%[g0]) dst_sel:DWORD dst_unused:UNUSED_PAD src0_sel:BYTE_1\n\t" \
	"v_cvt_f32_i32_sdwa v130, sext(%[g0]) dst_sel:DWORD dst_unused:UNUSED_PAD src0_sel:BYTE_2\n\t" \
	"v_cvt_f32_i32_sdwa v131, sext(%[g0]) dst_sel:DWORD dst_unused:UNUSED_PAD src0_sel:BYTE_3\n\t" \
	"v_cvt_f32_i32_sdwa v132, sext(%[g1]) dst_sel:DWORD dst_unused:UNUSED_PAD src0_sel:BYTE_0\n\t" \
	"v_cvt_f32_i32_sdwa v133, sext(%[g1]) dst_sel:DWORD dst_unused:UNUSED_PAD src0_sel:BYTE_1\n\t" \
	"v_cvt_f32_i32_sdwa v134, sext(%[g1]) dst_sel:DWORD dst_unused:UNUSED_PAD src0_sel:BYTE_2\n\t" \
	"v_cvt_f32_i32_sdwa v135, sext(%[g1]) dst_sel:DWORD dst_unused:UNUSED_PAD src0_sel:BYTE_3\n\t" \
	"v_cvt_f32_i32_sdwa v136, sext(%[g2]) dst_sel:DWORD dst_unused:UNUSED_PAD src0_sel:BYTE_0\n\t" \
	"v_cvt_f32_i32_sdwa v137, sext(%[g2]) dst_sel:DWORD dst_unused:UNUSED_PAD src0_sel:BYTE_1\n\t" \
	"v_cvt_f32_i32_sdwa v138, sext(%[g2]) dst_sel:DWORD dst_unused:UNUSED_PAD src0_sel:BYTE_2\n\t" \
	"v_cvt_f32_i32_sdwa v139, sext(%[g2]) dst_sel:DWORD dst_unused:UNUSED_PAD src0_sel:BYTE_3\n\t" \
	"v_cvt_f32_i32_sdwa v140, sext(%[g3]) dst_sel:DWORD dst_unused:UNUSED_PAD src0_sel:BYTE_0\n\t" \
	"v_cvt_f32_i32_sdwa v141, sext(%[g3]) dst_sel:DWORD dst_unused:UNUSED_PAD src0_sel:BYTE_1\n\t" \
	"v_cvt_f32_i32_sdwa v142, sext(%[g3]) dst_sel:DWORD dst_unused:UNUSED_PAD src0_sel:BYTE_2\n\t" \
	"v_cvt_f32_i32_sdwa v143, sext(%[g3]) dst_sel:DWORD dst_unused:UNUSED_PAD src0_sel:BYTE_3\n\t" \
	"s_branch .Lput_end_%=\n\t" \
	".Lput_3_%=:\n\t" \
	"v_cvt_f32_i32_sdwa v144, sext(%[g0]) dst_sel:DWORD dst_unused:UNUSED_PAD src0_sel:BYTE_0\n\t" \
	"v_cvt_f32_i32_sdwa v145, sext(%[g0]) dst_sel:DWORD dst_unused:UNUSED_PAD src0_sel:BYTE_1\n\t" \
	"v_cvt_f32_i32_sdwa v146, sext(%[g0]) dst_sel:DWORD dst_unused:UNUSED_PAD src0_sel:BYTE_2\n\t" \
	"v_cvt_f32_i32_sdwa v147, sext(%[g0]) dst_sel:DWORD dst_unused:UNUSED_PAD src0_sel:BYTE_3\n\t" \
	"v_cvt_f32_i32_sdwa v148, sext(%[g1]) dst_sel:DWORD dst_unused:UNUSED_PAD src0_sel:BYTE_0\n\t" \
	"v_cvt_f32_i32_sdwa v149, sext(%[g1]) dst_sel:DWORD dst_unused:UNUSED_PAD src0_sel:BYTE_1\n\t" \
	"v_cvt_f32_i32_sdwa v150, sext(%[g1]) dst_sel:DWORD dst_unused:UNUSED_PAD src0_sel:BYTE_2\n\t" \
	"v_cvt_f32_i32_sdwa v151, sext(%[g1]) dst_sel:DWORD dst_unused:UNUSED_PAD src0_sel:BYTE_3\n\t" \
	"v_cvt_f32_i32_sdwa v152, sext(%[g2]) dst_sel:DWORD dst_unused:UNUSED_PAD src0_sel:BYTE_0\n\t" \
	"v_cvt_f32_i32_sdwa v153, sext(%[g2]) dst_sel:DWORD dst_unused:UNUSED_PAD src0_sel:BYTE_1\n\t" \
	"v_cvt_f32_i32_sdwa v154, sext(%[g2]) dst_sel:DWORD dst_unused:UNUSED_PAD src0_sel:BYTE_2\n\t" \
	"v_cvt_f32_i32_sdwa v155, sext(%[g2]) dst_sel:DWORD dst_unused:UNUSED_PAD src0_sel:BYTE_3\n\t" \
	"v_cvt_f32_i32_sdwa v156, sext(%[g3]) dst_sel:DWORD dst_unused:UNUSED_PAD src0_sel:BYTE_0\n\t" \
	"v_cvt_f32_i32_sdwa v157, sext(%[g3]) dst_sel:DWORD dst_unused:UNUSED_PAD src0_sel:BYTE_1\n\t" \
	"v_cvt_f32_i32_sdwa v158, sext(%[g3]) dst_sel:DWORD dst_unused:UNUSED_PAD src0_sel:BYTE_2\n\t" \
	"v_cvt_f32_i32_sdwa v159, sext(%[g3]) dst_sel:DWORD dst_unused:UNUSED_PAD src0_sel:BYTE_3\n\t" \
	"s_branch .Lput_end_%=\n\t" \
	".Lput_4_%=:\n\t" \
	"v_cvt_f32_i32_sdwa v160, sext(%[g0]) dst_sel:DWORD dst_unused:UNUSED_PAD src0_sel:BYTE_0\n\t" \
	"v_cvt_f32_i32_sdwa v161, sext(%[g0]) dst_sel:DWORD dst_unused:UNUSED_PAD src0_sel:BYTE_1\n\t" \
	"v_cvt_f32_i32_sdwa v162, sext(%[g0]) dst_sel:DWORD dst_unused:UNUSED_PAD src0_sel:BYTE_2\n\t" \
	"v_cvt_f32_i32_sdwa v163, sext(%[g0]) dst_sel:DWORD dst_unused:UNUSED_PAD src0_sel:BYTE_3\n\t" \
	"v_cvt_f32_i32_sdwa v164, sext(%[g1]) dst_sel:DWORD dst_unused:UNUSED_PAD src0_sel:BYTE_0\n\t" \
	"v_cvt_f32_i32_sdwa v165, sext(%[g1]) dst_sel:DWORD dst_unused:UNUSED_PAD src0_sel:BYTE_1\n\t" \
	"v_cvt_f32_i32_sdwa v166, sext(%[g1]) dst_sel:DWORD dst_unused:UNUSED_PAD src0_sel:BYTE_2\n\t" \
	"v_cvt_f32_i32_sdwa v167, sext(%[g1]) dst_sel:DWORD dst_unused:UNUSED_PAD src0_sel:BYTE_3\n\t" \
	"v_cvt_f32_i32_sdwa v168, sext(%[g2]) dst_sel:DWORD dst_unused:UNUSED_PAD src0_sel:BYTE_0\n\t" \
	"v_cvt_f32_i32_sdwa v169, sext(%[g2]) dst_sel:DWORD dst_unused:UNUSED_PAD src0_sel:BYTE_1\n\t" \
	"v_cvt_f32_i32_sdwa v170, sext(%[g2]) dst_sel:DWORD dst_unused:UNUSED_PAD src0_sel:BYTE_2\n\t" \
	"v_cvt_f32_i32_sdwa v171, sext(%[g2]) dst_sel:DWORD dst_unused:UNUSED_PAD src0_sel:BYTE_3\n\t" \
	"v_cvt_f32_i32_sdwa v172, sext(%[g3]) dst_sel:DWORD dst_unused:UNUSED_PAD src0_sel:BYTE_0\n\t" \
	"v_cvt_f32_i32_sdwa v173, sext(%[g3]) dst_sel:DWORD dst_unused:UNUSED_PAD src0_sel:BYTE_1\n\t" \
	"v_cvt_f32_i32_sdwa v174, sext(%[g3]) dst_sel:DWORD dst_unused:UNUSED_PAD src0_sel:BYTE_2\n\t" \
	"v_cvt_f32_i32_sdwa v175, sext(%[g3]) dst_sel:DWORD dst_unused:UNUSED_PAD src0_sel:BYTE_3\n\t" \
	"s_branch .Lput_end_%=\n\t" \
	".Lput_5_%=:\n\t" \
	"v_cvt_f32_i32_sdwa v176, sext(%[g0]) dst_sel:DWORD dst_unused:UNUSED_PAD src0_sel:BYTE_0\n\t" \
	"v_cvt_f32_i32_sdwa v177, sext(%[g0]) dst_sel:DWORD dst_unused:UNUSED_PAD src0_sel:BYTE_1\n\t" \
	"v_cvt_f32_i32_sdwa v178, sext(%[g0]) dst_sel:DWORD dst_unused:UNUSED_PAD src0_sel:BYTE_2\n\t" \
	"v_cvt_f32_i32_sdwa v179, sext(%[g0]) dst_sel:DWORD dst_unused:UNUSED_PAD src0_sel:BYTE_3\n\t" \
	"v_cvt_f32_i32_sdwa v180, sext(%[g1]) dst_sel:DWORD dst_unused:UNUSED_PAD src0_sel:BYTE_0\n\t" \
	"v_cvt_f32_i32_sdwa v181, sext(%[g1]) dst_sel:DWORD dst_unused:UNUSED_PAD src0_sel:BYTE_1\n\t" \
	"v_cvt_f32_i32_sdwa v182, sext(%[g1]) dst_sel:DWORD dst_unused:UNUSED_PAD src0_sel:BYTE_2\n\t" \
	"v_cvt_f32_i32_sdwa v183, sext(%[g1]) dst_sel:DWORD dst_unused:UNUSED_PAD src0_sel:BYTE_3\n\t" \
	"v_cvt_f32_i32_sdwa v184, sext(%[g2]) dst_sel:DWORD dst_unused:UNUSED_PAD src0_sel:BYTE_0\n\t" \
	"v_cvt_f32_i32_sdwa v185, sext(%[g2]) dst_sel:DWORD dst_unused:UNUSED_PAD src0_sel:BYTE_1\n\t" \
	"v_cvt_f32_i32_sdwa v186, sext(%[g2]) dst_sel:DWORD dst_unused:UNUSED_PAD src0_sel:BYTE_2\n\t" \
	"v_cvt_f32_i32_sdwa v187, sext(%[g2]) dst_sel:DWORD dst_unused:UNUSED_PAD src0_sel:BYTE_3\n\t" \
	"v_cvt_f32_i32_sdwa v188, sext(%[g3]) dst_sel:DWORD dst_unused:UNUSED_PAD src0_sel:BYTE_0\n\t" \
	"v_cvt_f32_i32_sdwa v189, sext(%[g3]) dst_sel:DWORD dst_unused:UNUSED_PAD src0_sel:BYTE_1\n\t" \
	"v_cvt_f32_i32_sdwa v190, sext(%[g3]) dst_sel:DWORD dst_unused:UNUSED_PAD src0_sel:BYTE_2\n\t" \
	"v_cvt_f32_i32_sdwa v191, sext(%[g3]) dst_sel:DWORD dst_unused:UNUSED_PAD src0_sel:BYTE_3\n\t" \
	"s_branch .Lput_end_%=\n\t" \
	".Lput_6_%=:\n\t" \
	"v_cvt_f32_i32_sdwa v192, sext(%[g0]) dst_sel:DWORD dst_unused:UNUSED_PAD src0_sel:BYTE_0\n\t" \
	"v_cvt_f32_i32_sdwa v193, sext(%[g0]) dst_sel:DWORD dst_unused:UNUSED_PAD src0_sel:BYTE_1\n\t" \
	"v_cvt_f32_i32_sdwa v194, sext(%[g0]) dst_sel:DWORD dst_unused:UNUSED_PAD src0_sel:BYTE_2\n\t" \
	"v_cvt_f32_i32_sdwa v195, sext(%[g0]) dst_sel:DWORD dst_unused:UNUSED_PAD src0_sel:BYTE_3\n\t" \
	"v_cvt_f32_i32_sdwa v196, sext(%[g1]) dst_sel:DWORD dst_unused:UNUSED_PAD src0_sel:BYTE_0\n\t" \
	"v_cvt_f32_i32_sdwa v197, sext(%[g1]) dst_sel:DWORD dst_unused:UNUSED_PAD src0_sel:BYTE_1\n\t" \
	"v_cvt_f32_i32_sdwa v198, sext(%[g1]) dst_sel:DWORD dst_unused:UNUSED_PAD src0_sel:BYTE_2\n\t" \
	"v_cvt_f32_i32_sdwa v199, sext(%[g1]) dst_sel:DWORD dst_unused:UNUSED_PAD src0_sel:BYTE_3\n\t" \
	"v_cvt_f32_i32_sdwa v200, sext(%[g2]) dst_sel:DWORD dst_unused:UNUSED_PAD src0_sel:BYTE_0\n\t" \
	"v_cvt_f32_i32_sdwa v201, sext(%[g2]) dst_sel:DWORD dst_unused:UNUSED_PAD src0_sel:BYTE_1\n\t" \
	"v_cvt_f32_i32_sdwa v202, sext(%[g2]) dst_sel:DWORD dst_unused:UNUSED_PAD src0_sel:BYTE_2\n\t" \
	"v_cvt_f32_i32_sdwa v203, sext(%[g2]) dst_sel:DWORD dst_unused:UNUSED_PAD src0_sel:BYTE_3\n\t" \
	"v_cvt_f32_i32_sdwa v204, sext(%[g3]) dst_sel:DWORD dst_unused:UNUSED_PAD src0_sel:BYTE_0\n\t" \
	"v_cvt_f32_i32_sdwa v205, sext(%[g3]) dst_sel:DWORD dst_unused:UNUSED_PAD src0_sel:BYTE_1\n\t" \
	"v_cvt_f32_i32_sdwa v206, sext(%[g3]) dst_sel:DWORD dst_unused:UNUSED_PAD src0_sel:BYTE_2\n\t" \
	"v_cvt_f32_i32_sdwa v207, sext(%[g3]) dst_sel:DWORD dst_unused:UNUSED_PAD src0_sel:BYTE_3\n\t" \
	"s_branch .Lput_end_%=\n\t" \
	".Lput_7_%=:\n\t" \
	"v_cvt_f32_i32_sdwa v208, sext(%[g0]) dst_sel:DWORD dst_unused:UNUSED_PAD src0_sel:BYTE_0\n\t" \
	"v_cvt_f32_i32_sdwa v209, sext(%[g0]) dst_sel:DWORD dst_unused:UNUSED_PAD src0_sel:BYTE_1\n\t" \
	"v_cvt_f32_i32_sdwa v210, sext(%[g0]) dst_sel:DWORD dst_unused:UNUSED_PAD src0_sel:BYTE_2\n\t" \
	"v_cvt_f32_i32_sdwa v211, sext(%[g0]) dst_sel:DWORD dst_unused:UNUSED_PAD src0_sel:BYTE_3\n\t" \
	"v_cvt_f32_i32_sdwa v212, sext(%[g1]) dst_sel:DWORD dst_unused:UNUSED_PAD src0_sel:BYTE_0\n\t" \
	"v_cvt_f32_i32_sdwa v213, sext(%[g1]) dst_sel:DWORD dst_unused:UNUSED_PAD src0_sel:BYTE_1\n\t" \
	"v_cvt_f32_i32_sdwa v214, sext(%[g1]) dst_sel:DWORD dst_unused:UNUSED_PAD src0_sel:BYTE_2\n\t" \
	"v_cvt_f32_i32_sdwa v215, sext(%[g1]) dst_sel:DWORD dst_unused:UNUSED_PAD src0_sel:BYTE_3\n\t" \
	"v_cvt_f32_i32_sdwa v216, sext(%[g2]) dst_sel:DWORD dst_unused:UNUSED_PAD src0_sel:BYTE_0\n\t" \
	"v_cvt_f32_i32_sdwa v217, sext(%[g2]) dst_sel:DWORD dst_unused:UNUSED_PAD src0_sel:BYTE_1\n\t" \
	"v_cvt_f32_i32_sdwa v218, sext(%[g2]) dst_sel:DWORD dst_unused:UNUSED_PAD src0_sel:BYTE_2\n\t" \
	"v_cvt_f32_i32_sdwa v219, sext(%[g2]) dst_sel:DWORD dst_unused:UNUSED_PAD src0_sel:BYTE_3\n\t" \
	"v_cvt_f32_i32_sdwa v220, sext(%[g3]) dst_sel:DWORD dst_unused:UNUSED_PAD src0_sel:BYTE_0\n\t" \
	"v_cvt_f32_i32_sdwa v221, sext(%[g3]) dst_sel:DWORD dst_unused:UNUSED_PAD src0_sel:BYTE_1\n\t" \
	"v_cvt_f32_i32_sdwa v222, sext(%[g3]) dst_sel:DWORD dst_unused:UNUSED_PAD src0_sel:BYTE_2\n\t" \
	"v_cvt_f32_i32_sdwa v223, sext(%[g3]) dst_sel:DWORD dst_unused:UNUSED_PAD src0_sel:BYTE_3\n\t" \
	"s_branch .Lput_end_%=\n\t" \
	".Lput_8_%=:\n\t" \
	"v_cvt_f32_i32_sdwa v224, sext(%[g0]) dst_sel:DWORD dst_unused:UNUSED_PAD src0_sel:BYTE_0\n\t" \
	"v_cvt_f32_i32_sdwa v225, sext(%[g0]) dst_sel:DWORD dst_unused:UNUSED_PAD src0_sel:BYTE_1\n\t" \
	"v_cvt_f32_i32_sdwa v226, sext(%[g0]) dst_sel:DWORD dst_unused:UNUSED_PAD src0_sel:BYTE_2\n\t" \
	"v_cvt_f32_i32_sdwa v227, sext(%[g0]) dst_sel:DWORD dst_unused:UNUSED_PAD src0_sel:BYTE_3\n\t" \
	"v_cvt_f32_i32_sdwa v228, sext(%[g1]) dst_sel:DWORD dst_unused:UNUSED_PAD src0_sel:BYTE_0\n\t" \
	"v_cvt_f32_i32_sdwa v229, sext(%[g1]) dst_sel:DWORD dst_unused:UNUSED_PAD src0_sel:BYTE_1\n\t" \
	"v_cvt_f32_i32_sdwa v230, sext(%[g1]) dst_sel:DWORD dst_unused:UNUSED_PAD src0_sel:BYTE_2\n\t" \
	"v_cvt_f32_i32_sdwa v231, sext(%[g1]) dst_sel:DWORD dst_unused:UNUSED_PAD src0_sel:BYTE_3\n\t" \
	"v_cvt_f32_i32_sdwa v232, sext(%[g2]) dst_sel:DWORD dst_unused:UNUSED_PAD src0_sel:BYTE_0\n\t" \
	"v_cvt_f32_i32_sdwa v233, sext(%[g2]) dst_sel:DWORD dst_unused:UNUSED_PAD src0_sel:BYTE_1\n\t" \
	"v_cvt_f32_i32_sdwa v234, sext(%[g2]) dst_sel:DWORD dst_unused:UNUSED_PAD src0_sel:BYTE_2\n\t" \
	"v_cvt_f32_i32_sdwa v235, sext(%[g2]) dst_sel:DWORD dst_unused:UNUSED_PAD src0_sel:BYTE_3\n\t" \
	"v_cvt_f32_i32_sdwa v236, sext(%[g3]) dst_sel:DWORD dst_unused:UNUSED_PAD src0_sel:BYTE_0\n\t" \
	"v_cvt_f32_i32_sdwa v237, sext(%[g3]) dst_sel:DWORD dst_unused:UNUSED_PAD src0_sel:BYTE_1\n\t" \
	"v_cvt_f32_i32_sdwa v238, sext(%[g3]) dst_sel:DWORD dst_unused:UNUSED_PAD src0_sel:BYTE_2\n\t" \
	"v_cvt_f32_i32_sdwa v239, sext(%[g3]) dst_sel:DWORD dst_unused:UNUSED_PAD src0_sel:BYTE_3\n\t" \
	"s_branch .Lput_end_%=\n\t" \
	".Lput_9_%=:\n\t" \
	"v_cvt_f32_i32_sdwa v240, sext(%[g0]) dst_sel:DWORD dst_unused:UNUSED_PAD src0_sel:BYTE_0\n\t" \
	"v_cvt_f32_i32_sdwa v241, sext(%[g0]) dst_sel:DWORD dst_unused:UNUSED_PAD src0_sel:BYTE_1\n\t" \
	"v_cvt_f32_i32_sdwa v242, sext(%[g0]) dst_sel:DWORD dst_unused:UNUSED_PAD src0_sel:BYTE_2\n\t" \
	"v_cvt_f32_i32_sdwa v243, sext(%[g0]) dst_sel:DWORD dst_unused:UNUSED_PAD src0_sel:BYTE_3\n\t" \
	"v_cvt_f32_i32_sdwa v244, sext(%[g1]) dst_sel:DWORD dst_unused:UNUSED_PAD src0_sel:BYTE_0\n\t" \
	"v_cvt_f32_i32_sdwa v245, sext(%[g1]) dst_sel:DWORD dst_unused:UNUSED_PAD src0_sel:BYTE_1\n\t" \
	"v_cvt_f32_i32_sdwa v246, sext(%[g1]) dst_sel:DWORD dst_unused:UNUSED_PAD src0_sel:BYTE_2\n\t" \
	"v_cvt_f32_i32_sdwa v247, sext(%[g1]) dst_sel:DWORD dst_unused:UNUSED_PAD src0_sel:BYTE_3\n\t" \
	"v_cvt_f32_i32_sdwa v248, sext(%[g2]) dst_sel:DWORD dst_unused:UNUSED_PAD src0_sel:BYTE_0\n\t" \
	"v_cvt_f32_i32_sdwa v249, sext(%[g2]) dst_sel:DWORD dst_unused:UNUSED_PAD src0_sel:BYTE_1\n\t" \
	"v_cvt_f32_i32_sdwa v250, sext(%[g2]) dst_sel:DWORD dst_unused:UNUSED_PAD src0_sel:BYTE_2\n\t" \
	"v_cvt_f32_i32_sdwa v251, sext(%[g2]) dst_sel:DWORD dst_unused:UNUSED_PAD src0_sel:BYTE_3\n\t" \
	"v_cvt_f32_i32_sdwa v252, sext(%[g3]) dst_sel:DWORD dst_unused:UNUSED_PAD src0_sel:BYTE_0\n\t" \
	"v_cvt_f32_i32_sdwa v253, sext(%[g3]) dst_sel:DWORD dst_unused:UNUSED_PAD src0_sel:BYTE_1\n\t" \
	"v_cvt_f32_i32_sdwa v254, sext(%[g3]) dst_sel:DWORD dst_unused:UNUSED_PAD src0_sel:BYTE_2\n\t" \
	"v_cvt_f32_i32_sdwa v255, sext(%[g3]) dst_sel:DWORD dst_unused:UNUSED_PAD src0_sel:BYTE_3\n\t" \
	"s_branch .Lput_end_%=\n\t" \
	".Lput_end_%=:\n\t"
#define ROTWIN_PUT_F32_ASM \
	"s_getpc_b64 vcc\n\t" \
	".Lput_pc_%=:\n\t" \
	"s_mul_i32 %[tmp], %[rot], (.Lput_1_%= - .Lput_0_%=)\n\t" \
	"s_add_u32 %[tmp], %[tmp], (.Lput_0_%= - .Lput_pc_%=)\n\t" \
	"s_add_u32 vcc_lo, vcc_lo, %[tmp]\n\t" \
	"s_addc_u32 vcc_hi, vcc_hi, 0\n\t" \
	"s_setpc_b64 vcc\n\t" \
	".Lput_0_%=:\n\t" \
	"v_mov_b32 v96, %[f0]\n\t" \
	"v_mov_b32 v97, %[f1]\n\t" \
	"v_mov_b32 v98, %[f2]\n\t" \
	"v_mov_b32 v99, %[f3]\n\t" \
	"v_mov_b32 v100, %[f4]\n\t" \
	"v_mov_b32 v101, %[f5]\n\t" \
	"v_mov_b32 v102, %[f6]\n\t" \
	"v_mov_b32 v103, %[f7]\n\t" \
	"v_mov_b32 v104, %[f8]\n\t" \
	"v_mov_b32 v105, %[f9]\n\t" \
	"v_mov_b32 v106, %[f10]\n\t" \
	"v_mov_b32 v107, %[f11]\n\t" \
	"v_mov_b32 v108, %[f12]\n\t" \
	"v_mov_b32 v109, %[f13]\n\t" \
	"v_mov_b32 v110, %[f14]\n\t" \
	"v_mov_b32 v111, %[f15]\n\t" \
	"s_branch .Lput_end_%=\n\t" \
	".Lput_1_%=:\n\t" \
	"v_mov_b32 v112, %[f0]\n\t" \
	"v_mov_b32 v113, %[f1]\n\t" \
	"v_mov_b32 v114, %[f2]\n\t" \
	"v_mov_b32 v115, %[f3]\n\t" \
	"v_mov_b32 v116, %[f4]\n\t" \
	"v_mov_b32 v117, %[f5]\n\t" \
	"v_mov_b32 v118, %[f6]\n\t" \
	"v_mov_b32 v119, %[f7]\n\t" \
	"v_mov_b32 v120, %[f8]\n\t" \
	"v_mov_b32 v121, %[f9]\n\t" \
	"v_mov_b32 v122, %[f10]\n\t" \
	"v_mov_b32 v123, %[f11]\n\t" \
	"v_mov_b32 v124, %[f12]\n\t" \
	"v_mov_b32 v125, %[f13]\n\t" \
	"v_mov_b32 v126, %[f14]\n\t" \
	"v_mov_b32 v127, %[f15]\n\t" \
	"s_branch .Lput_end_%=\n\t" \
	".Lput_2_%=:\n\t" \
	"v_mov_b32 v128, %[f0]\n\t" \
	"v_mov_b32 v129, %[f1]\n\t" \
	"v_mov_b32 v130, %[f2]\n\t" \
	"v_mov_b32 v131, %[f3]\n\t" \
	"v_mov_b32 v132, %[f4]\n\t" \
	"v_mov_b32 v133, %[f5]\n\t" \
	"v_mov_b32 v134, %[f6]\n\t" \
	"v_mov_b32 v135, %[f7]\n\t" \
	"v_mov_b32 v136, %[f8]\n\t" \
	"v_mov_b32 v137, %[f9]\n\t" \
	"v_mov_b32 v138, %[f10]\n\t" \
	"v_mov_b32 v139, %[f11]\n\t" \
	"v_mov_b32 v140, %[f12]\n\t" \
	"v_mov_b32 v141, %[f13]\n\t" \
	"v_mov_b32 v142, %[f14]\n\t" \
	"v_mov_b32 v143, %[f15]\n\t" \
	"s_branch .Lput_end_%=\n\t" \
	".Lput_3_%=:\n\t" \
	"v_mov_b32 v144, %[f0]\n\t" \
	"v_mov_b32 v145, %[f1]\n\t" \
	"v_mov_b32 v146, %[f2]\n\t" \
	"v_mov_b32 v147, %[f3]\n\t" \
	"v_mov_b32 v148, %[f4]\n\t" \
	"v_mov_b32 v149, %[f5]\n\t" \
	"v_mov_b32 v150, %[f6]\n\t" \
	"v_mov_b32 v151, %[f7]\n\t" \
	"v_mov_b32 v152, %[f8]\n\t" \
	"v_mov_b32 v153, %[f9]\n\t" \
	"v_mov_b32 v154, %[f10]\n\t" \
	"v_mov_b32 v155, %[f11]\n\t" \
	"v_mov_b32 v156, %[f12]\n\t" \
	"v_mov_b32 v157, %[f13]\n\t" \
	"v_mov_b32 v158, %[f14]\n\t" \
	"v_mov_b32 v159, %[f15]\n\t" \
	"s_branch .Lput_end_%=\n\t" \
	".Lput_4_%=:\n\t" \
	"v_mov_b32 v160, %[f0]\n\t" \
	"v_mov_b32 v161, %[f1]\n\t" \
	"v_mov_b32 v162, %[f2]\n\t" \
	"v_mov_b32 v163, %[f3]\n\t" \
	"v_mov_b32 v164, %[f4]\n\t" \
	"v_mov_b32 v165, %[f5]\n\t" \
	"v_mov_b32 v166, %[f6]\n\t" \
	"v_mov_b32 v167, %[f7]\n\t" \
	"v_mov_b32 v168, %[f8]\n\t" \
	"v_mov_b32 v169, %[f9]\n\t" \
	"v_mov_b32 v170, %[f10]\n\t" \
	"v_mov_b32 v171, %[f11]\n\t" \
	"v_mov_b32 v172, %[f12]\n\t" \
	"v_mov_b32 v173, %[f13]\n\t" \
	"v_mov_b32 v174, %[f14]\n\t" \
	"v_mov_b32 v175, %[f15]\n\t" \
	"s_branch .Lput_end_%=\n\t" \
	".Lput_5_%=:\n\t" \
	"v_mov_b32 v176, %[f0]\n\t" \
	"v_mov_b32 v177, %[f1]\n\t" \
	"v_mov_b32 v178, %[f2]\n\t" \
	"v_mov_b32 v179, %[f3]\n\t" \
	"v_mov_b32 v180, %[f4]\n\t" \
	"v_mov_b32 v181, %[f5]\n\t" \
	"v_mov_b32 v182, %[f6]\n\t" \
	"v_mov_b32 v183, %[f7]\n\t" \
	"v_mov_b32 v184, %[f8]\n\t" \
	"v_mov_b32 v185, %[f9]\n\t" \
	"v_mov_b32 v186, %[f10]\n\t" \
	"v_mov_b32 v187, %[f11]\n\t" \
	"v_mov_b32 v188, %[f12]\n\t" \
	"v_mov_b32 v189, %[f13]\n\t" \
	"v_mov_b32 v190, %[f14]\n\t" \
	"v_mov_b32 v191, %[f15]\n\t" \
	"s_branch .Lput_end_%=\n\t" \
	".Lput_6_%=:\n\t" \
	"v_mov_b32 v192, %[f0]\n\t" \
	"v_mov_b32 v193, %[f1]\n\t" \
	"v_mov_b32 v194, %[f2]\n\t" \
	"v_mov_b32 v195, %[f3]\n\t" \
	"v_mov_b32 v196, %[f4]\n\t" \
	"v_mov_b32 v197, %[f5]\n\t" \
	"v_mov_b32 v198, %[f6]\n\t" \
	"v_mov_b32 v199, %[f7]\n\t" \
	"v_mov_b32 v200, %[f8]\n\t" \
	"v_mov_b32 v201, %[f9]\n\t" \
	"v_mov_b32 v202, %[f10]\n\t" \
	"v_mov_b32 v203, %[f11]\n\t" \
	"v_mov_b32 v204, %[f12]\n\t" \
	"v_mov_b32 v205, %[f13]\n\t" \
	"v_mov_b32 v206, %[f14]\n\t" \
	"v_mov_b32 v207, %[f15]\n\t" \
	"s_branch .Lput_end_%=\n\t" \
	".Lput_7_%=:\n\t" \
	"v_mov_b32 v208, %[f0]\n\t" \
	"v_mov_b32 v209, %[f1]\n\t" \
	"v_mov_b32 v210, %[f2]\n\t" \
	"v_mov_b32 v211, %[f3]\n\t" \
	"v_mov_b32 v212, %[f4]\n\t" \
	"v_mov_b32 v213, %[f5]\n\t" \
	"v_mov_b32 v214, %[f6]\n\t" \
	"v_mov_b32 v215, %[f7]\n\t" \
	"v_mov_b32 v216, %[f8]\n\t" \
	"v_mov_b32 v217, %[f9]\n\t" \
	"v_mov_b32 v218, %[f10]\n\t" \
	"v_mov_b32 v219, %[f11]\n\t" \
	"v_mov_b32 v220, %[f12]\n\t" \
	"v_mov_b32 v221, %[f13]\n\t" \
	"v_mov_b32 v222, %[f14]\n\t" \
	"v_mov_b32 v223, %[f15]\n\t" \
	"s_branch .Lput_end_%=\n\t" \
	".Lput_8_%=:\n\t" \
	"v_mov_b32 v224, %[f0]\n\t" \
	"v_mov_b32 v225, %[f1]\n\t" \
	"v_mov_b32 v226, %[f2]\n\t" \
	"v_mov_b32 v227, %[f3]\n\t" \
	"v_mov_b32 v228, %[f4]\n\t" \
	"v_mov_b32 v229, %[f5]\n\t" \
	"v_mov_b32 v230, %[f6]\n\t" \
	"v_mov_b32 v231, %[f7]\n\t" \
	"v_mov_b32 v232, %[f8]\n\t" \
	"v_mov_b32 v233, %[f9]\n\t" \
	"v_mov_b32 v234, %[f10]\n\t" \
	"v_mov_b32 v235, %[f11]\n\t" \
	"v_mov_b32 v236, %[f12]\n\t" \
	"v_mov_b32 v237, %[f13]\n\t" \
	"v_mov_b32 v238, %[f14]\n\t" \
	"v_mov_b32 v239, %[f15]\n\t" \
	"s_branch .Lput_end_%=\n\t" \
	".Lput_9_%=:\n\t" \
	"v_mov_b32 v240, %[f0]\n\t" \
	"v_mov_b32 v241, %[f1]\n\t" \
	"v_mov_b32 v242, %[f2]\n\t" \
	"v_mov_b32 v243, %[f3]\n\t" \
	"v_mov_b32 v244, %[f4]\n\t" \
	"v_mov_b32 v245, %[f5]\n\t" \
	"v_mov_b32 v246, %[f6]\n\t" \
	"v_mov_b32 v247, %[f7]\n\t" \
	"v_mov_b32 v248, %[f8]\n\t" \
	"v_mov_b32 v249, %[f9]\n\t" \
	"v_mov_b32 v250, %[f10]\n\t" \
	"v_mov_b32 v251, %[f11]\n\t" \
	"v_mov_b32 v252, %[f12]\n\t" \
	"v_mov_b32 v253, %[f13]\n\t" \
	"v_mov_b32 v254, %[f14]\n\t" \
	"v_mov_b32 v255, %[f15]\n\t" \
	"s_branch .Lput_end_%=\n\t" \
	".Lput_end_%=:\n\t"
#define ROTWIN_FIR_ACC_ASM \
	"ds_read_b128 v[80:83], %[addr] offset:0\n\t" \
	"ds_read_b128 v[84:87], %[addr] offset:16\n\t" \
	"s_getpc_b64 vcc\n\t" \
	".Lfira_pc_%=:\n\t" \
	"s_mul_i32 %[tmp], %[rot], (.Lfira_1_%= - .Lfira_0_%=)\n\t" \
	"s_add_u32 %[tmp], %[tmp], (.Lfira_0_%= - .Lfira_pc_%=)\n\t" \
	"s_add_u32 vcc_lo, vcc_lo, %[tmp]\n\t" \
	"s_addc_u32 vcc_hi, vcc_hi, 0\n\t" \
	"s_setpc_b64 vcc\n\t" \
	".Lfira_0_%=:\n\t" \
	"ds_read_b128 v[88:91], %[addr] offset:32\n\t" \
	"s_waitcnt lgkmcnt(2)\n\t" \
	"v_accvgpr_read_b32 v92, a96\n\t" \
	"v_accvgpr_read_b32 v93, a97\n\t" \
	"v_accvgpr_read_b32 v94, a98\n\t" \
	"v_accvgpr_read_b32 v95, a99\n\t" \
	"v_pk_mul_f32 v[92:93], v[92:93], v[80:81] op_sel:[0,0] op_sel_hi:[1,0]\n\t" \
	"v_pk_mul_f32 v[94:95], v[94:95], v[80:81] op_sel:[0,1] op_sel_hi:[1,1]\n\t" \
	"v_pk_add_f32 %[acc], %[acc], v[92:93]\n\t" \
	"v_accvgpr_read_b32 v92, a100\n\t" \
	"v_accvgpr_read_b32 v93, a101\n\t" \
	"v_pk_add_f32 %[acc], %[acc], v[94:95]\n\t" \
	"v_accvgpr_read_b32 v94, a102\n\t" \
	"v_accvgpr_read_b32 v95, a103\n\t" \
	"v_pk_mul_f32 v[92:93], v[92:93], v[82:83] op_sel:[0,0] op_sel_hi:[1,0]\n\t" \
	"v_pk_mul_f32 v[94:95], v[94:95], v[82:83] op_sel:[0,1] op_sel_hi:[1,1]\n\t" \
	"v_pk_add_f32 %[acc], %[acc], v[92:93]\n\t" \
	"v_pk_add_f32 %[acc], %[acc], v[94:95]\n\t" \
	"ds_read_b128 v[80:83], %[addr] offset:48\n\t" \
	"s_waitcnt lgkmcnt(2)\n\t" \
	"v_accvgpr_read_b32 v92, a104\n\t" \
	"v_accvgpr_read_b32 v93, a105\n\t" \
	"v_accvgpr_read_b32 v94, a106\n\t" \
	"v_accvgpr_read_b32 v95, a107\n\t" \
	"v_pk_mul_f32 v[92:93], v[92:93], v[84:85] op_sel:[0,0] op_sel_hi:[1,0]\n\t" \
	"v_pk_mul_f32 v[94:95], v[94:95], v[84:85] op_sel:[0,1] op_sel_hi:[1,1]\n\t" \
	"v_pk_add_f32 %[acc], %[acc], v[92:93]\n\t" \
	"v_accvgpr_read_b32 v92, a108\n\t" \
	"v_accvgpr_read_b32 v93, a109\n\t" \
	"v_pk_add_f32 %[acc], %[acc], v[94:95]\n\t" \
	"v_accvgpr_read_b32 v94, a110\n\t" \
	"v_accvgpr_read_b32 v95, a111\n\t" \
	"v_pk_mul_f32 v[92:93], v[92:93], v[86:87] op_sel:[0,0] op_sel_hi:[1,0]\n\t" \
	"v_pk_mul_f32 v[94:95], v[94:95], v[86:87] op_sel:[0,1] op_sel_hi:[1,1]\n\t" \
	"v_pk_add_f32 %[acc], %[acc], v[92:93]\n\t" \
	"v_pk_add_f32 %[acc], %[acc], v[94:95]\n\t" \
	"ds_read_b128 v[84:87], %[addr] offset:64\n\t" \
	"s_waitcnt lgkmcnt(2)\n\t" \
	"v_accvgpr_read_b32 v92, a112\n\t" \
	"v_accvgpr_read_b32 v93, a113\n\t" \
	"v_accvgpr_read_b32 v94, a114\n\t" \
	"v_accvgpr_read_b32 v95, a115\n\t" \
	"v_pk_mul_f32 v[92:93], v[92:93], v[88:89] op_sel:[0,0] op_sel_hi:[1,0]\n\t" \
	"v_pk_mul_f32 v[94:95], v[94:95], v[88:89] op_sel:[0,1] op_sel_hi:[1,1]\n\t" \
	"v_pk_add_f32 %[acc], %[acc], v[92:93]\n\t" \
	"v_accvgpr_read_b32 v92, a116\n\t" \
	"v_accvgpr_read_b32 v93, a117\n\t" \
	"v_pk_add_f32 %[acc], %[acc], v[94:95]\n\t" \
	"v_accvgpr_read_b32 v94, a118\n\t" \
	"v_accvgpr_read_b32 v95, a119\n\t" \
	"v_pk_mul_f32 v[92:93], v[92:93], v[90:91] op_sel:[0,0] op_sel_hi:[1,0]\n\t" \
	"v_pk_mul_f32 v[94:95], v[94:95], v[90:91] op_sel:[0,1] op_sel_hi:[1,1]\n\t" \
	"v_pk_add_f32 %[acc], %[acc], v[92:93]\n\t" \
	"v_pk_add_f32 %[acc], %[acc], v[94:95]\n\t" \
	"ds_read_b128 v[88:91], %[addr] offset:80\n\t" \
	"s_waitcnt lgkmcnt(2)\n\t" \
	"v_accvgpr_read_b32 v92, a120\n\t" \
	"v_accvgpr_read_b32 v93, a121\n\t" \
	"v_accvgpr_read_b32 v94, a122\n\t" \
	"v_accvgpr_read_b32 v95, a123\n\t" \
	"v_pk_mul_f32 v[92:93], v[92:93], v[80:81] op_sel:[0,0] op_sel_hi:[1,0]\n\t" \
	"v_pk_mul_f32 v[94:95], v[94:95], v[80:81] op_sel:[0,1] op_sel_hi:[1,1]\n\t" \
	"v_pk_add_f32 %[acc], %[acc], v[92:93]\n\t" \
	"v_accvgpr_read_b32 v92, a124\n\t" \
	"v_accvgpr_read_b32 v93, a125\n\t" \
	"v_pk_add_f32 %[acc], %[acc], v[94:95]\n\t" \
	"v_accvgpr_read_b32 v94, a126\n\t" \
	"v_accvgpr_read_b32 v95, a127\n\t" \
	"v_pk_mul_f32 v[92:93], v[92:93], v[82:83] op_sel:[0,0] op_sel_hi:[1,0]\n\t" \
	"v_pk_mul_f32 v[94:95], v[94:95], v[82:83] op_sel:[0,1] op_sel_hi:[1,1]\n\t" \
	"v_pk_add_f32 %[acc], %[acc], v[92:93]\n\t" \
	"v_pk_add_f32 %[acc], %[acc], v[94:95]\n\t" \
	"ds_read_b128 v[80:83], %[addr] offset:96\n\t" \
	"s_waitcnt lgkmcnt(2)\n\t" \
	"v_accvgpr_read_b32 v92, a128\n\t" \
	"v_accvgpr_read_b32 v93, a129\n\t" \
	"v_accvgpr_read_b32 v94, a130\n\t" \
	"v_accvgpr_read_b32 v95, a131\n\t" \
	"v_pk_mul_f32 v[92:93], v[92:93], v[84:85] op_sel:[0,0] op_sel_hi:[1,0]\n\t" \
	"v_pk_mul_f32 v[94:95], v[94:95], v[84:85] op_sel:[0,1] op_sel_hi:[1,1]\n\t" \
	"v_pk_add_f32 %[acc], %[acc], v[92:93]\n\t" \
	"v_accvgpr_read_b32 v92, a132\n\t" \
	"v_accvgpr_read_b32 v93, a133\n\t" \
	"v_pk_add_f32 %[acc], %[acc], v[94:95]\n\t" \
	"v_accvgpr_read_b32 v94, a134\n\t" \
	"v_accvgpr_read_b32 v95, a135\n\t" \
	"v_pk_mul_f32 v[92:93], v[92:93], v[86:87] op_sel:[0,0] op_sel_hi:[1,0]\n\t" \
	"v_pk_mul_f32 v[94:95], v[94:95], v[86:87] op_sel:[0,1] op_sel_hi:[1,1]\n\t" \
	"v_pk_add_f32 %[acc], %[acc], v[92:93]\n\t" \
	"v_pk_add_f32 %[acc], %[acc], v[94:95]\n\t" \
	"ds_read_b128 v[84:87], %[addr] offset:112\n\t" \
	"s_waitcnt lgkmcnt(2)\n\t" \
	"v_accvgpr_read_b32 v92, a136\n\t" \
	"v_accvgpr_read_b32 v93, a137\n\t" \
	"v_accvgpr_read_b32 v94, a138\n\t" \
	"v_accvgpr_read_b32 v95, a139\n\t" \
	"v_pk_mul_f32 v[92:93], v[92:93], v[88:89] op_sel:[0,0] op_sel_hi:[1,0]\n\t" \
	"v_pk_mul_f32 v[94:95], v[94:95], v[88:89] op_sel:[0,1] op_sel_hi:[1,1]\n\t" \
	"v_pk_add_f32 %[acc], %[acc], v[92:93]\n\t" \
	"v_accvgpr_read_b32 v92, a140\n\t" \
	"v_accvgpr_read_b32 v93, a141\n\t" \
	"v_pk_add_f32 %[acc], %[acc], v[94:95]\n\t" \
	"v_accvgpr_read_b32 v94, a142\n\t" \
	"v_accvgpr_read_b32 v95, a143\n\t" \
	"v_pk_mul_f32 v[92:93], v[92:93], v[90:91] op_sel:[0,0] op_sel_hi:[1,0]\n\t" \
	"v_pk_mul_f32 v[94:95], v[94:95], v[90:91] op_sel:[0,1] op_sel_hi:[1,1]\n\t" \
	"v_pk_add_f32 %[acc], %[acc], v[92:93]\n\t" \
	"v_pk_add_f32 %[acc], %[acc], v[94:95]\n\t" \
	"ds_read_b128 v[88:91], %[addr] offset:128\n\t" \
	"s_waitcnt lgkmcnt(2)\n\t" \
	"v_accvgpr_read_b32 v92, a144\n\t" \
	"v_accvgpr_read_b32 v93, a145\n\t" \
	"v_accvgpr_read_b32 v94, a146\n\t" \
	"v_accvgpr_read_b32 v95, a147\n\t" \
	"v_pk_mul_f32 v[92:93], v[92:93], v[80:81] op_sel:[0,0] op_sel_hi:[1,0]\n\t" \
	"v_pk_mul_f32 v[94:95], v[94:95], v[80:81] op_sel:[0,1] op_sel_hi:[1,1]\n\t" \
	"v_pk_add_f32 %[acc], %[acc], v[92:93]\n\t" \
	"v_accvgpr_read_b32 v92, a148\n\t" \
	"v_accvgpr_read_b32 v93, a149\n\t" \
	"v_pk_add_f32 %[acc], %[acc], v[94:95]\n\t" \
	"v_accvgpr_read_b32 v94, a150\n\t" \
	"v_accvgpr_read_b32 v95, a151\n\t" \
	"v_pk_mul_f32 v[92:93], v[92:93], v[82:83] op_sel:[0,0] op_sel_hi:[1,0]\n\t" \
	"v_pk_mul_f32 v[94:95], v[94:95], v[82:83] op_sel:[0,1] op_sel_hi:[1,1]\n\t" \
	"v_pk_add_f32 %[acc], %[acc], v[92:93]\n\t" \
	"v_pk_add_f32 %[acc], %[acc], v[94:95]\n\t" \
	"ds_read_b128 v[80:83], %[addr] offset:144\n\t" \
	"s_waitcnt lgkmcnt(2)\n\t" \
	"v_accvgpr_read_b32 v92, a152\n\t" \
	"v_accvgpr_read_b32 v93, a153\n\t" \
	"v_accvgpr_read_b32 v94, a154\n\t" \
	"v_accvgpr_read_b32 v95, a155\n\t" \
	"v_pk_mul_f32 v[92:93], v[92:93], v[84:85] op_sel:[0,0] op_sel_hi:[1,0]\n\t" \
	"v_pk_mul_f32 v[94:95], v[94:95], v[84:85] op_sel:[0,1] op_sel_hi:[1,1]\n\t" \
	"v_pk_add_f32 %[acc], %[acc], v[92:93]\n\t" \
	"v_accvgpr_read_b32 v92, a156\n\t" \
	"v_accvgpr_read_b32 v93, a157\n\t" \
	"v_pk_add_f32 %[acc], %[acc], v[94:95]\n\t" \
	"v_accvgpr_read_b32 v94, a158\n\t" \
	"v_accvgpr_read_b32 v95, a159\n\t" \
	"v_pk_mul_f32 v[92:93], v[92:93], v[86:87] op_sel:[0,0] op_sel_hi:[1,0]\n\t" \
	"v_pk_mul_f32 v[94:95], v[94:95], v[86:87] op_sel:[0,1] op_sel_hi:[1,1]\n\t" \
// ... 6015 lines not shown
```

meteor_demod_amd/csrc/rotwin_body.h:

```cpp
#ifndef MDEMOD_ROTWIN_BODY_H
#define MDEMOD_ROTWIN_BODY_H

#include <hip/hip_runtime.h>
#include <stdint.h>

#include "demod_internal.h"
#include "demod_device.h"
#include "clock_jump.h"

#pragma clang fp contract(off)

#ifndef ROT_OQ_SYNC
#define ROT_OQ_SYNC 1
#endif
typedef float rot_sinlut_t;

namespace {

template <int FMT> struct RFmt;
template <> struct RFmt<16> { typedef uint32_t sample_t; enum { GDW = 4 }; };
template <> struct RFmt<8>  { typedef uint16_t sample_t; enum { GDW = 2 }; };
template <> struct RFmt<32> { typedef float2   sample_t; enum { GDW = 8 }; };

template <int FMT> struct RGran { uint32_t w[RFmt<FMT>::GDW]; };

template <int FMT>
__device__ __forceinline__ RGran<FMT>
rot_fetch(const typename RFmt<FMT>::sample_t *src, int m0, int n)
{
	typedef typename RFmt<FMT>::sample_t sample_t;
	RGran<FMT> g;
	if (m0 + 3 < n) {
		__builtin_memcpy(&g, src + m0, sizeof(g));
	} else {
		sample_t s[4];
#pragma unroll
		for (int u = 0; u < 4; u++) {
			if (m0 + u < n) s[u] = src[m0 + u];
			else __builtin_memset(&s[u], 0, sizeof(s[u]));
		}
		__builtin_memcpy(&g, s, sizeof(g));
	}
	return g;
}

__device__ __forceinline__ uint32_t
rot_mad24(uint32_t a, uint32_t b, uint32_t c)
{
	uint32_t r;
	asm("v_mad_u32_u24 %0, %1, %2, %3" : "=v"(r) : "v"(a), "s"(b), "v"(c));
	return r;
}

template <int K>
__device__ __forceinline__ float
blind_steps(float p, float f)
{
#pragma unroll
	for (int k = 0; k < K; k++) p = p + f;
	return p;
}

typedef int rot_i4 __attribute__((ext_vector_type(4)));
typedef const __attribute__((address_space(3))) rot_i4 *rot_clktab_t;
struct RotClockConsts { int k_safe, steps_need, interp; float f_hi; uint32_t magic; float inv; const cj_sched *jump; rot_clktab_t tab; };
template <int KS>
__device__ __forceinline__ void
rot_clock_fast(const RotClockConsts &K, float thr, int v_end, float &t_phase, float t_freq, int &isub, int &v_cur, int &bank, bool &fired, int jidx = -1)
{
	int k_safe = KS ? KS : K.k_safe;
	const int interp = K.interp;
	const bool jump = KS == 0 && jidx >= 0 && K.jump[jidx < 0 ? 0 : jidx].nb > 0;
	const cj_sched &J = K.jump[jidx < 0 ? 0 : jidx];
	const bool fast = (KS == 109 ? (t_phase > CJ109_P_LO && t_phase < CJ109_P_HI)
	                   : jump    ? (t_phase > J.floor && t_phase < J.hi)
	                             : (t_phase < thr - (float)k_safe * K.f_hi - 1e-3f))
	                  && (v_cur + (jump ? J.need : K.steps_need) < v_end);
	if (fast) {
		float p = t_phase;
		if (KS == 109) k_safe = clock_jump_109(p, t_freq, thr, K.inv);
		else if (KS) p = blind_steps<KS>(p, t_freq);
		else if (jump) k_safe = clock_jump_run(p, t_freq, thr, K.f_hi, K.inv, J);
		else {
			int k = k_safe;
			for (; k >= 16; k -= 16) p = blind_steps<16>(p, t_freq);
			if (k & 8) p = blind_steps<8>(p, t_freq);
			if (k & 4) p = blind_steps<4>(p, t_freq);
			if (k & 2) p = blind_steps<2>(p, t_freq);
			if (k & 1) p = p + t_freq;
		}
		const float p1 = p + t_freq, p2 = p1 + t_freq, p3 = p2 + t_freq, p4 = p3 + t_freq;
		const bool c1 = p1 >= thr, c2 = p2 >= thr, c3 = p3 >= thr, c4 = p4 >= thr;
		float ph = c3 ? p3 : p4;
		ph = c2 ? p2 : ph;
		ph = c1 ? p1 : ph;
		t_phase = ph;
		if ((KS == 14 || KS == 6) || (KS == 0 && K.tab)) {
			const uint32_t off = ((uint32_t)isub << 6) + (c1 ? 0u : 16u) + (c2 ? 0u : 16u) + (c3 ? 0u : 16u);
			const rot_i4 e = *reinterpret_cast<rot_clktab_t>(reinterpret_cast<const __attribute__((address_space(3))) unsigned char *>(K.tab) + off);
			v_cur += e.x;
			isub = e.z;
			bank = e.w;
		} else {
			const uint32_t w = (uint32_t)(isub + k_safe + 1 + (c1 ? 0 : 1) + (c2 ? 0 : 1) + (c3 ? 0 : 1));
			const uint32_t q = (interp == 1) ? w : __umulhi(w, K.magic);
			const int isub_new = (int)(w - q * (uint32_t)interp);
			v_cur += (int)q + (isub_new > 0 ? 1 : 0) - (isub > 0 ? 1 : 0);
			const int fire_sub = (isub_new == 0) ? interp - 1 : isub_new - 1;
			bank = interp - 1 - fire_sub;
			isub = isub_new;
		}
		fired = c4;
	}
}


template <class W, int FMT, int OQPSK, int KS, int LUT = 0>
__device__ __forceinline__ void
rotwin_demod(const DemodLaunch &L)
{
	typedef typename RFmt<FMT>::sample_t sample_t;
	constexpr int kBack = W::kBack, SLIDE = W::SLIDE, AMAX = W::AMAX, BLOCK = W::BLOCK, NCH = W::NW / W::SLIDE, GPS = W::SLIDE / 4;
	constexpr int NST = GPS * W::DEPTH;
	static_assert(W::DEPTH >= W::MAXSL, "a loop iteration may slide MAXSL times");
	constexpr int ROTN = W::ROTN, RING = W::RING, RGR = RING / 8;
	constexpr bool GATHER = W::GATHER;
	static_assert(RING == 32 || RING == 16, "output ring");
	constexpr int RS = W::REGSLOTS;
#ifndef ROT_PRIO
#define ROT_PRIO 1
#endif
#ifndef ROT_PRIO_LEVEL
#define ROT_PRIO_LEVEL 2
#endif
	constexpr int PRIO = ROT_PRIO;

	extern __shared__ __attribute__((aligned(16))) unsigned char lds[];
	float *ctab = reinterpret_cast<float *>(lds);
	float *lut = ctab + L.ctab_floats;
	enum { S_GAIN, S_BIAS_RE, S_BIAS_IM, S_PHASE, S_FREQ, S_ERR, S_FLAGS, S_TPREV, S_INPHASE, S_EVCALL, S_FIRSTLOCK, S_LASTV, S_COUNT };
	static_assert(S_COUNT == MDEMOD_RW_STATE_SLOTS, "host LDS sizing");
	float *sl = lut + 32 + (threadIdx.x >> 6) * (S_COUNT * 64) + (threadIdx.x & 63);
	int *sli = reinterpret_cast<int *>(sl);
	uint4 *stage = reinterpret_cast<uint4 *>(lut + 32 + (BLOCK / 64) * (S_COUNT * 64)) + threadIdx.x;
	const uint32_t ctab_addr = (uint32_t)(uintptr_t)(__attribute__((address_space(3))) unsigned char *)lds;
	W win;
	rot_sinlut_t *sintab = reinterpret_cast<rot_sinlut_t *>(stage - threadIdx.x + BLOCK * RGR);
	if constexpr (LUT) md_sin_lut_fill(sintab, (int)threadIdx.x, BLOCK);
	win.setup(ctab_addr + (uint32_t)(reinterpret_cast<unsigned char *>(stage - threadIdx.x + BLOCK * RGR) - lds) + (LUT ? MDEMOD_SIN_LUT_BYTES : 0));
	rot_i4 *clktab = reinterpret_cast<rot_i4 *>(reinterpret_cast<unsigned char *>(stage - threadIdx.x + BLOCK * RGR) + (LUT ? MDEMOD_SIN_LUT_BYTES : 0));

	const DemodConsts &C = L.c;
	const uint32_t stream = blockIdx.x * blockDim.x + threadIdx.x;
	const bool valid = stream < L.n_streams;

	for (uint32_t i = threadIdx.x; i < L.ctab_floats; i += blockDim.x) ctab[i] = L.ctab[i];
	if (threadIdx.x < 32) lut[threadIdx.x] = L.tanh_lut[threadIdx.x];
	const bool has_clktab = KS != 109 && C.clock_tab != nullptr;
	if (has_clktab)
		for (int i = (int)threadIdx.x; i < 4 * C.interp; i += (int)blockDim.x) clktab[i] = reinterpret_cast<const rot_i4 *>(C.clock_tab)[i];

	int n = 0;
	const sample_t *src = nullptr;
	if (valid) {
		n = (int)(L.n_samples_arr ? L.n_samples_arr[stream] : L.n_samples);
		const uint64_t off = L.iq_offset ? L.iq_offset[stream] : (uint64_t)stream * L.iq_stride;
		src = reinterpret_cast<const sample_t *>(L.iq) + off;
	}
	const int v_end = kBack + n;
	const int interp = C.interp;

	float t_phase = 0.0f, t_freq = C.t_center;
	int dual_state = 1;
	float r_gain = 1.0f, r_bias_re = 0.0f, r_bias_im = 0.0f, r_phase = 0.0f, r_freq = 0.0f;
	float r_err = 1000.0f, r_tprev = 0.0f;
	int r_flags = 0, r_lastv = -1;
	auto ld_err = [&]() -> float { return (RS & 1) ? r_err : sl[S_ERR * 64]; };
	auto st_err = [&](float v) { if (RS & 1) r_err = v; else sl[S_ERR * 64] = v; };
	auto ld_tprev = [&]() -> float { return (RS & 2) ? r_tprev : sl[S_TPREV * 64]; };
	auto st_tprev = [&](float v) { if (RS & 2) r_tprev = v; else sl[S_TPREV * 64] = v; };
	auto ld_flags = [&]() -> int { return (RS & 4) ? r_flags : sli[S_FLAGS * 64]; };
	auto st_flags = [&](int v) { if (RS & 4) r_flags = v; else sli[S_FLAGS * 64] = v; };
	auto ld_lastv = [&]() -> int { return (RS & 8) ? r_lastv : sli[S_LASTV * 64]; };
	auto st_lastv = [&](int v) { if (RS & 8) r_lastv = v; else sli[S_LASTV * 64] = v; };
	{
		float err = 1000.0f, t_prev = 0.0f, inph = 0.0f;
		int fl = MDEMOD_FLAG_UPDOWN_POS | (1 << MDEMOD_FLAG_DUAL_SHIFT);
		if (valid) {
			r_gain = L.st.agc_gain[stream]; r_bias_re = L.st.agc_bias_re[stream]; r_bias_im = L.st.agc_bias_im[stream];
			r_phase = L.st.pll_phase[stream]; r_freq = L.st.pll_freq[stream]; err = L.st.pll_err[stream];
			fl = L.st.flags[stream];
			t_phase = L.st.t_phase[stream]; t_freq = L.st.t_freq[stream]; t_prev = L.st.t_prev[stream];
			inph = L.st.inphase[stream];
		}
		dual_state = (fl >> MDEMOD_FLAG_DUAL_SHIFT) & 3;
		st_err(err);
		st_flags(fl & 7);
		st_tprev(t_prev); sl[S_INPHASE * 64] = inph;
		sli[S_EVCALL * 64] = 0; sli[S_FIRSTLOCK * 64] = -1; st_lastv(-1);
	}

	const float2 *hist_in = reinterpret_cast<const float2 *>(L.st.hist) + (size_t)(valid ? stream : 0) * kBack;
	if constexpr (!GATHER) {
		const float2 *hist = hist_in;
#pragma unroll 1
		for (int c = 0; c < kBack / SLIDE; c++) win.put_history(hist + c * SLIDE, valid, __builtin_amdgcn_readfirstlane(c));
#pragma unroll 1
		for (int c = 0; c < NCH - kBack / SLIDE; c++) {
			RGran<FMT> g[GPS];
#pragma unroll
			for (int i = 0; i < GPS; i++) g[i] = rot_fetch<FMT>(src, SLIDE * c + 4 * i, n);
			win.put_init(g, __builtin_amdgcn_readfirstlane(kBack / SLIDE + c));
		}
	}
	int g_load = (W::NW - kBack) / 4;
	RGran<FMT> stg[GATHER ? 1 : NST];
	if constexpr (!GATHER) {
#pragma unroll
		for (int i = 0; i < NST; i++) stg[i] = rot_fetch<FMT>(src, 4 * (g_load + i), n);
		g_load += NST;
	}

	__syncthreads();

	int rot = 0;
	int slot = 1;
	int base = 0;
	int isub = 0, bank = interp - 1;
	bool fired = false;
	bool done = !valid || n == 0;
	constexpr int V_DONE = 0x3FFFFFFF;
	int v_cur = done ? V_DONE : kBack - 1;
	uint32_t sym_call = 0;
	RotClockConsts K;
	K.k_safe = C.step_safe; K.f_hi = C.step_fmax; K.magic = C.interp_magic; K.interp = C.interp; K.inv = C.step_inv;
	K.steps_need = ((KS == 109 ? CJ109_MAX_STEPS : C.step_safe) + 4 + C.interp - 1) / C.interp;
	K.jump = C.jump;
	K.tab = has_clktab ? (rot_clktab_t)clktab : (rot_clktab_t)0;

	int n_wave_max = n;
	for (int o = 32; o > 0; o >>= 1) {
		const int other = __shfl_xor(n_wave_max, o);
		n_wave_max = other > n_wave_max ? other : n_wave_max;
	}
	n_wave_max = __builtin_amdgcn_readfirstlane(n_wave_max);
	const uint64_t guard64 = 4ull * (uint64_t)(n_wave_max + kBack) * (uint64_t)interp + 4096ull;
	uint32_t guard = guard64 > 0xFFFFFFFFull ? 0xFFFFFFFFu : (uint32_t)guard64;
#ifdef ROT_EXP_TIMING
	uint64_t tacc[5] = { 0, 0, 0, 0, 0 }, tlast = clock64();
	uint32_t n_iter = 0, n_fir = 0, n_slide = 0, n_wslow = 0;
#define ROT_TICK(i) do { const uint64_t t_ = clock64(); tacc[i] += t_ - tlast; tlast = t_; } while (0)
#else
#define ROT_TICK(i) do { } while (0)
#endif
	do {
		ROT_TICK(4);
		if (!fired && !done) {
			const float thr = OQPSK ? (float)dual_state * MD_PI_F : MD_TWO_PI_F;
			rot_clock_fast<KS>(K, thr, v_end, t_phase, t_freq, isub, v_cur, bank, fired);
			while (!fired && !done) {
				if (isub == 0) {
					if (v_cur + 1 >= v_end) { done = true; v_cur = V_DONE; break; }
					v_cur++;
				}
				t_phase = t_phase + t_freq;
				bank = interp - 1 - isub;
				isub = (isub + 1 == interp) ? 0 : isub + 1;
				if (t_phase >= thr) fired = true;
			}
		}
		if constexpr (GATHER) if (md_all(v_cur == V_DONE)) break;
		ROT_TICK(0);
#ifdef ROT_EXP_TIMING
		n_iter++;
#endif

		bool all_done = false;
		if constexpr (!GATHER)
#pragma unroll
		for (int r = 0; r < W::MAXSL; r++) {
			const int a_now = v_cur - kBack - base;
			if (md_all(a_now >= SLIDE)) {
				if (md_all(v_cur == V_DONE)) { all_done = true; break; }
				RGran<FMT> g[GPS];
#pragma unroll
				for (int i = 0; i < GPS; i++) g[i] = stg[i];
				win.put(g, __builtin_amdgcn_readfirstlane(rot));
				rot = __builtin_amdgcn_readfirstlane((rot == ROTN - 1) ? 0 : rot + 1);
				base = __builtin_amdgcn_readfirstlane(base + SLIDE);
#pragma unroll
				for (int i = 0; i + GPS < NST; i++) stg[i] = stg[i + GPS];
				const int m_new = 4 * g_load;
				if (md_all(m_new + SLIDE - 1 < n)) {
#pragma unroll
					for (int i = 0; i < GPS; i++) __builtin_memcpy(&stg[NST - GPS + i], src + m_new + 4 * i, sizeof(RGran<FMT>));
				} else {
#pragma unroll
					for (int i = 0; i < GPS; i++) stg[NST - GPS + i] = rot_fetch<FMT>(src, m_new + 4 * i, n);
				}
				g_load += GPS;
			}
		}
		if (all_done) break;

		ROT_TICK(1);
		const int a = v_cur - kBack - base;
		if (fired && (GATHER || a <= AMAX) && (!(OQPSK && ROT_OQ_SYNC) || dual_state == slot)) {
			fired = false;
			cf32 y;
			if constexpr (GATHER) win.fir_gather(ctab_addr, src, hist_in, v_cur, n, bank, C, y.re, y.im);
			else win.fir(ctab_addr, a, bank, C, __builtin_amdgcn_readfirstlane(rot), y.re, y.im);
			if (PRIO) __builtin_amdgcn_s_setprio(ROT_PRIO_LEVEL);
			ROT_TICK(2);
#ifdef ROT_EXP_TIMING
			n_fir++;
#endif

			y = md_agc<(KS == 14 && !OQPSK && LUT)>(y, r_gain, r_bias_re, r_bias_im);
			uint32_t fl = (uint32_t)ld_flags();
			PllWord pll;
			pll.phase = r_phase; pll.freq = r_freq;
			pll.err = ld_err();

			float sn, cs;
			if constexpr (LUT) {
				sn = md_sin_from_code_lut(sintab, md_turn_code<false>(-pll.phase));
				cs = md_sin_from_code_lut(sintab, md_turn_code<false>((float)((double)(-pll.phase) + MD_HALF_PI_D)));
			} else {
				sn = md_fast_sin<false>(-pll.phase);
				cs = md_fast_cos<false>(-pll.phase);
			}
			bool emit = true;
			float out_re, out_im;
			if (OQPSK) {
				float inphase = sl[S_INPHASE * 64];
				const int rail = ROT_OQ_SYNC ? slot : dual_state;
				if (rail == 1) { inphase = y.re * cs - y.im * sn; emit = false; sl[S_INPHASE * 64] = inphase; }
				out_re = inphase;
				out_im = y.re * sn + y.im * cs;
				dual_state = 3 - rail;
			} else {
				out_re = y.re * cs - y.im * sn;
				out_im = y.re * sn + y.im * cs;
			}
			md_nco_advance<true>(pll.phase, pll.freq);

			if (emit) {
				const bool again = (v_cur == ld_lastv());
				st_lastv(v_cur);
				if (__builtin_expect(md_any(again), 0)) { if (again) sym_call--; }
				float t_prev = ld_tprev();
				md_timing_update(t_phase, t_freq, t_prev, C.t_alpha, C.t_beta, C.t_center, C.t_maxdev, out_im);
				st_tprev(t_prev);
			}
			rot_clock_fast<KS>(K, OQPSK ? (float)dual_state * MD_PI_F : MD_TWO_PI_F, v_end, t_phase, t_freq, isub, v_cur, bank, fired,
			                   OQPSK ? (ROT_OQ_SYNC ? 2 - slot : -1) : 0);
#ifdef ROT_EXP_TIMING
			if (!fired) n_slide++;
			if (md_any(!fired)) n_wslow++;
#endif
			if (emit) {
				uint32_t first = 0;
				const uint32_t changed = md_pll_update_packed(pll, fl, lut, C.pll_alpha, C.pll_beta, C.pll_fmax, out_re, out_im, first);
				if (__builtin_expect(changed != 0, 0)) {
					if (first) sli[S_FIRSTLOCK * 64] = (int)sym_call;
					const int ev_call = sli[S_EVCALL * 64];
					if (ev_call < MDEMOD_MAX_LOCK_EVENTS) {
						mdemod_lock_event ev;
						ev.symbol = L.st.n_symbols[stream] + sym_call; ev.locked = (int)(fl & 1u); ev.pad = 0;
						L.st.events[(size_t)stream * MDEMOD_MAX_LOCK_EVENTS + ev_call] = ev;
					}
					sli[S_EVCALL * 64] = ev_call + 1;
				}
				const uint32_t sym = (uint32_t)(md_quantise(out_re) & 0xFF) | ((uint32_t)(md_quantise(out_im) & 0xFF) << 8);
				const uint32_t k = sym_call & (uint32_t)(RING - 1);
				reinterpret_cast<uint16_t *>(stage + (k >> 3) * BLOCK)[k & 7u] = (uint16_t)sym;
				sym_call++;
				if (__builtin_expect((sym_call & (uint32_t)(RING - 1)) == 0, 0)) {
					int8_t *soft_out = L.soft + (size_t)stream * L.soft_stride * 2;
					if (__builtin_expect(sym_call <= L.soft_cap, 1)) {
						int8_t *dst = soft_out + 2 * (size_t)(sym_call - RING);
#pragma unroll
						for (int g4 = 0; g4 < RGR; g4++) {
							const uint4 qv = stage[g4 * BLOCK];
							__builtin_memcpy(dst + 16 * g4, &qv, 16);
							asm volatile("" ::: "memory");
						}
					} else {
						fl |= 8;
						for (uint32_t i = 0; i < (uint32_t)RING && sym_call - RING + i < L.soft_cap; i++)
							*reinterpret_cast<uint16_t *>(soft_out + 2 * (size_t)(sym_call - RING + i)) =
							    reinterpret_cast<const uint16_t *>(stage + (i >> 3) * BLOCK)[i & 7u];
					}
				}
			}
			r_phase = pll.phase; r_freq = pll.freq;
			st_err(pll.err);
			st_flags((int)fl);
			if (PRIO == 1) __builtin_amdgcn_s_setprio(0);
			ROT_TICK(3);
		}
		if (OQPSK && ROT_OQ_SYNC) slot = __builtin_amdgcn_readfirstlane(3 - slot);
	} while (--guard);
#ifdef ROT_EXP_TIMING
	for (int o = 32; o > 0; o >>= 1) n_slide += __shfl_xor(n_slide, o);
	if (blockIdx.x == 100 && threadIdx.x == 0)
		printf("ROT_TIMING iters %u firs %u (lanes left to the stepping loop: %u of the wave's, in %u firings) cycles: clock %llu slide %llu fir %llu scalar %llu latch %llu\n", n_iter, n_fir, n_slide, n_wslow,
		       (unsigned long long)tacc[0], (unsigned long long)tacc[1], (unsigned long long)tacc[2], (unsigned long long)tacc[3], (unsigned long long)tacc[4]);
#endif

	if (guard == 0) st_flags(ld_flags() | 8);

	uint32_t stream_e = stream;
	asm volatile("" : "+v"(stream_e));
	int8_t *soft_e = L.soft + (size_t)stream_e * L.soft_stride * 2;
	int overflow = (ld_flags() >> 3) & 1;

	if (valid) {
		const uint32_t r = sym_call & (uint32_t)(RING - 1), sb = sym_call - r;
		for (uint32_t g = 0; g < (r >> 3); g++) {
			if (sb + 8 * g + 8 <= L.soft_cap) { const uint4 qv = stage[g * BLOCK]; __builtin_memcpy(soft_e + 2 * (size_t)(sb + 8 * g), &qv, 16); }
			else for (uint32_t i = 0; i < 8; i++) {
				if (sb + 8 * g + i < L.soft_cap) *reinterpret_cast<uint16_t *>(soft_e + 2 * (size_t)(sb + 8 * g + i)) = reinterpret_cast<const uint16_t *>(stage + g * BLOCK)[i];
				else overflow = 1;
			}
		}
		for (uint32_t i = r & ~7u; i < r; i++) {
			if (sb + i < L.soft_cap) *reinterpret_cast<uint16_t *>(soft_e + 2 * (size_t)(sb + i)) = reinterpret_cast<const uint16_t *>(stage + (i >> 3) * BLOCK)[i & 7u];
			else overflow = 1;
		}
	}

	if (valid) {
		const int fl = ld_flags();
		L.st.agc_gain[stream_e] = r_gain; L.st.agc_bias_re[stream_e] = r_bias_re; L.st.agc_bias_im[stream_e] = r_bias_im;
		L.st.pll_phase[stream_e] = r_phase; L.st.pll_freq[stream_e] = r_freq; L.st.pll_err[stream_e] = ld_err();
		L.st.flags[stream_e] = (fl & 7) | (dual_state << MDEMOD_FLAG_DUAL_SHIFT);
		L.st.t_phase[stream_e] = t_phase; L.st.t_freq[stream_e] = t_freq; L.st.t_prev[stream_e] = ld_tprev();
		L.st.inphase[stream_e] = sl[S_INPHASE * 64];
		const uint64_t nsym0 = L.st.n_symbols[stream_e];
		const int first_lock_call = sli[S_FIRSTLOCK * 64];
		L.st.n_samples[stream_e] += (uint64_t)n;
		L.st.n_symbols[stream_e] = nsym0 + sym_call;
		if (first_lock_call >= 0) L.st.first_lock[stream_e] = (int64_t)(nsym0 + (uint32_t)first_lock_call);
		L.st.sym_this_call[stream_e] = sym_call;
		L.st.ev_this_call[stream_e] = (uint32_t)sli[S_EVCALL * 64];
		L.st.overflow[stream_e] = overflow;

		float2 *hist = reinterpret_cast<float2 *>(L.st.hist) + (size_t)stream_e * kBack;
		for (int k = 0; k < kBack; k++) {
			const int idx = n + k;
			float2 h;
			if (idx < kBack) h = hist[idx];
			else {
				const sample_t raw = src[idx - kBack];
				if constexpr (FMT == 16) h = make_float2((float)(int)(int16_t)(raw & 0xFFFFu), (float)((int)raw >> 16));
				else if constexpr (FMT == 8) h = make_float2((float)((int)(raw & 0xFFu) - 128), (float)((int)(raw >> 8) - 128));
				else h = raw;
			}
			hist[k] = h;
		}
	}
}


}

#endif
```

Measured before the change: 266,300.

## Keep slide state in SGPRs inside put asm and trim scalar/vector bookkeeping

Moves the ring rotation and base advance into the window-put assembly so they stay in scalar registers, dropping the readfirstlane sequences around each slide. The FIR skip flags are now computed from wave ballots, and the accumulator is zeroed inside the FIR asm. A precomputed fast-path end bound is hoisted out of the clock step. Loop constants are pinned in VGPRs, and the LDS state address is forced into a VGPR. The intent is to cut scalar/vector transfer overhead and per-symbol instruction count, at the cost of extra VGPR pressure and more coupling between the asm and the C++ code.

Result: faster. 270,000, median of 6 (+1.4%).

```diff
diff --git a/meteor_demod_amd/csrc/demod_kernel_gat.hip b/meteor_demod_amd/csrc/demod_kernel_gat.hip
--- a/meteor_demod_amd/csrc/demod_kernel_gat.hip
+++ b/meteor_demod_amd/csrc/demod_kernel_gat.hip
@@ -29,7 +29,7 @@
 struct WinG {
 	static constexpr int G = GFmt<FMT>::G, kTaps = KT, kBack = KT - 1, AMAX = G - 1, NS = KT + AMAX, NW = 4 * ((NS + 3) / 4), SLIDE = 4, MAXSL = 1, DEPTH = 1,
 	                     BLOCK = MDEMOD_RW_BLOCK, ROTN = 1, RING = 32, REGSLOTS = 0;
-	static constexpr bool GATHER = true;
+	static constexpr bool GATHER = true, SCALAR_SLIDE = false, VCONST = false;
 	static_assert(NS % G == 0 && NS / G <= 36, "whole 16-byte loads, and few enough of them to stay in registers");
 	typedef typename RFmt<FMT>::sample_t sample_t;
 	__device__ __forceinline__ void setup(uint32_t) {}
diff --git a/meteor_demod_amd/csrc/demod_kernel_rot.hip b/meteor_demod_amd/csrc/demod_kernel_rot.hip
--- a/meteor_demod_amd/csrc/demod_kernel_rot.hip
+++ b/meteor_demod_amd/csrc/demod_kernel_rot.hip
@@ -1,4 +1,5 @@
 #include "rotwin_body.h"
+#include "rot_fir_bounds.h"
 #include "hip_host.h"
 #ifdef ROTWIN_ASM_HEADER
 #include ROTWIN_ASM_HEADER
@@ -8,7 +9,7 @@
 
 namespace {
 
-static_assert(ROTWIN_NCH * 8 == 80, "window = ten chunks of eight");
+static_assert(ROTWIN_NCH * 8 == 80 && ROTWIN_SLIDE == 8, "window = ten chunks of eight, a slide brings one");
 
 
 __device__ __forceinline__ void
@@ -17,9 +18,9 @@
 	int tmp;
 #if ROTWIN_PK == 1 || ROTWIN_PK == 3
 	typedef float pair_t __attribute__((ext_vector_type(2)));
-	pair_t acc = { 0.0f, 0.0f }, p0, p1;
+	pair_t acc, p0, p1;
 	asm volatile(ROTWIN_FIR_ASM
-	             : [acc] "+v"(acc), [p0] "=&v"(p0), [p1] "=&v"(p1), [tmp] "=&s"(tmp)
+	             : [acc] "=&v"(acc), [p0] "=&v"(p0), [p1] "=&v"(p1), [tmp] "=&s"(tmp)
 	             : [addr] "v"(row_addr), [rot] "s"(rot), [flags] "s"(flags)
 	             : "vcc", "scc", ROTWIN_COEF_CLOBBERS);
 	re = acc.x; im = acc.y;
@@ -32,51 +33,59 @@
 #endif
 }
 
-template <int FMT> __device__ __forceinline__ void rot_put(const RGran<FMT> &a, const RGran<FMT> &b, int q);
+template <int FMT> __device__ __forceinline__ void rot_put(const RGran<FMT> &a, const RGran<FMT> &b, int &q, int &base);
 template <> __device__ __forceinline__ void
-rot_put<16>(const RGran<16> &a, const RGran<16> &b, int q)
+rot_put<16>(const RGran<16> &a, const RGran<16> &b, int &q, int &base)
 {
 	int tmp;
 	asm volatile(ROTWIN_PUT_S16_ASM
-	             : [tmp] "=&s"(tmp)
+	             : [tmp] "=&s"(tmp), [rot] "+s"(q), [base] "+s"(base)
 	             : [g0] "v"(a.w[0]), [g1] "v"(a.w[1]), [g2] "v"(a.w[2]), [g3] "v"(a.w[3]),
-	               [g4] "v"(b.w[0]), [g5] "v"(b.w[1]), [g6] "v"(b.w[2]), [g7] "v"(b.w[3]), [rot] "s"(q)
+	               [g4] "v"(b.w[0]), [g5] "v"(b.w[1]), [g6] "v"(b.w[2]), [g7] "v"(b.w[3])
 	             : "vcc", "scc", "v255", "memory");
 }
 template <> __device__ __forceinline__ void
-rot_put<8>(const RGran<8> &a, const RGran<8> &b, int q)
+rot_put<8>(const RGran<8> &a, const RGran<8> &b, int &q, int &base)
 {
 	const uint32_t g0 = a.w[0] ^ 0x80808080u, g1 = a.w[1] ^ 0x80808080u, g2 = b.w[0] ^ 0x80808080u, g3 = b.w[1] ^ 0x80808080u;
 	int tmp;
 	asm volatile(ROTWIN_PUT_U8_ASM
-	             : [tmp] "=&s"(tmp)
-	             : [g0] "v"(g0), [g1] "v"(g1), [g2] "v"(g2), [g3] "v"(g3), [rot] "s"(q)
+	             : [tmp] "=&s"(tmp), [rot] "+s"(q), [base] "+s"(base)
+	             : [g0] "v"(g0), [g1] "v"(g1), [g2] "v"(g2), [g3] "v"(g3)
 	             : "vcc", "scc", "v255", "memory");
 }
 __device__ __forceinline__ void
+rot_put_floats(const uint32_t (&f)[16], int &q, int &base)
+{
+	int tmp;
+	asm volatile(ROTWIN_PUT_F32_ASM
+	             : [tmp] "=&s"(tmp), [rot] "+s"(q), [base] "+s"(base)
+	             : [f0] "v"(f[0]), [f1] "v"(f[1]), [f2] "v"(f[2]), [f3] "v"(f[3]), [f4] "v"(f[4]), [f5] "v"(f[5]), [f6] "v"(f[6]), [f7] "v"(f[7]),
+	               [f8] "v"(f[8]), [f9] "v"(f[9]), [f10] "v"(f[10]), [f11] "v"(f[11]), [f12] "v"(f[12]), [f13] "v"(f[13]), [f14] "v"(f[14]), [f15] "v"(f[15])
+	             : "vcc", "scc", "v255", "memory");
+}
+__device__ __forceinline__ void
 rot_put_floats(const uint32_t (&f)[16], int q)
 {
-	int tmp;
-	asm volatile(ROTWIN_PUT_F32_ASM
-	             : [tmp] "=&s"(tmp)
-	             : [f0] "v"(f[0]), [f1] "v"(f[1]), [f2] "v"(f[2]), [f3] "v"(f[3]), [f4] "v"(f[4]), [f5] "v"(f[5]), [f6] "v"(f[6]), [f7] "v"(f[7]),
-	               [f8] "v"(f[8]), [f9] "v"(f[9]), [f10] "v"(f[10]), [f11] "v"(f[11]), [f12] "v"(f[12]), [f13] "v"(f[13]), [f14] "v"(f[14]), [f15] "v"(f[15]),
-	               [rot] "s"(q)
-	             : "vcc", "scc", "v255", "memory");
+	int base = 0;
+	rot_put_floats(f, q, base);
 }
 template <> __device__ __forceinline__ void
-rot_put<32>(const RGran<32> &a, const RGran<32> &b, int q)
+rot_put<32>(const RGran<32> &a, const RGran<32> &b, int &q, int &base)
 {
 	uint32_t f[16];
 #pragma unroll
 	for (int i = 0; i < 8; i++) { f[i] = a.w[i]; f[8 + i] = b.w[i]; }
-	rot_put_floats(f, q);
-}
-
-template <int FMT, int COMPACT = 0, int BLK = MDEMOD_RW_BLOCK>
+	rot_put_floats(f, q, base);
+}
+
+template <int FMT, int COMPACT = 0, int BLK = MDEMOD_RW_BLOCK, int VC = 0>
 struct WinF {
 	static constexpr int kTaps = 65, kBack = 64, NW = 80, SLIDE = 8, AMAX = NW - kTaps, MAXSL = 1, DEPTH = 1, BLOCK = BLK, ROTN = NW / SLIDE, RING = 32;
 	static constexpr bool GATHER = false;
+	static constexpr bool SCALAR_SLIDE = true;
+	static constexpr bool VCONST = VC != 0;
+	static_assert(SLIDE == ROTWIN_SLIDE && ROTN == ROTWIN_NCH, "the slide's assembly counts for itself");
 	__device__ __forceinline__ void setup(uint32_t) {}
 #ifndef ROT_REGSLOTS
 #define ROT_REGSLOTS 0
@@ -94,8 +103,9 @@
 		}
 		rot_put_floats(f, q);
 	}
-	__device__ static __forceinline__ void put(const RGran<FMT> (&g)[2], int q) { rot_put<FMT>(g[0], g[1], q); }
+	__device__ static __forceinline__ void put(const RGran<FMT> (&g)[2], int q) { int base = 0; rot_put<FMT>(g[0], g[1], q, base); }
 	__device__ static __forceinline__ void put_init(const RGran<FMT> (&g)[2], int q) { put(g, q); }
+	__device__ static __forceinline__ void slide(const RGran<FMT> (&g)[2], int &rot, int &base) { rot_put<FMT>(g[0], g[1], rot, base); }
 	__device__ static __forceinline__ void fir(uint32_t ctab_addr, int a, int bank, const DemodConsts &C, int rot, float &re, float &im)
 	{
 		const int o = AMAX - a;
@@ -103,15 +113,17 @@
 		if (COMPACT) row_addr = rot_mad24((uint32_t)(bank * 4 + (o & 3)), 4u * (uint32_t)C.ctab_row_stride, ctab_addr + 4u * (uint32_t)(o & ~3));
 		else row_addr = rot_mad24(rot_mad24((uint32_t)a, (uint32_t)C.interp, (uint32_t)bank), 4u * (uint32_t)C.ctab_row_stride, ctab_addr);
 		static_assert(AMAX == 15, "two bits of a / 4");
-		const int lo1 = md_all(a >= 8) ? 2 : 0, hi1 = md_all(a < 8) ? 1 : 3;
-		const int q_lo = md_all(a >= 4 * (lo1 + 1)) ? lo1 + 1 : lo1, q_hi = md_all(a < 4 * hi1) ? hi1 - 1 : hi1;
-		const int flags = ((1 << q_lo) - 1) | (((1 << (3 - q_hi)) - 1) << 3);
+		const uint64_t ex = __builtin_amdgcn_ballot_w64(true);
+		const RotFirQ q = rot_fir_q(ex, __builtin_amdgcn_ballot_w64(a >= 4), __builtin_amdgcn_ballot_w64(a >= 8), __builtin_amdgcn_ballot_w64(a >= 12));
+		int q_hi = q.q_hi;
+		asm("" : "+s"(q_hi));
+		const int flags = rot_fir_flags(q.q_lo, q_hi);
 #ifdef ROT_EXP_NOSKIP
 		int f0 = __builtin_amdgcn_readfirstlane(flags);
 		asm volatile("s_and_b32 %0, %0, 0" : "+s"(f0) : : "scc");
 		rot_fir(row_addr, rot, f0, re, im);
 #else
-		rot_fir(row_addr, rot, __builtin_amdgcn_readfirstlane(flags), re, im);
+		rot_fir(row_addr, rot, flags, re, im);
 #endif
 	}
 };
@@ -171,7 +183,7 @@
 struct WinH {
 	static constexpr int NR = 10, SLIDE = 8, NW = SLIDE * (NR + NA), kTaps = NA == 10 ? 129 : 65, kBack = kTaps - 1, AMAX = NW - kTaps, MAXSL = MSL, DEPTH = MSL,
 	                     BLOCK = BLK, ROTN = NR, RING = 32, REGSLOTS = 0;
-	static constexpr bool GATHER = false;
+	static constexpr bool GATHER = false, SCALAR_SLIDE = false, VCONST = false;
 	static_assert((NA == 10 || NA == 2 || NA == 5) && AMAX == (NA == 5 ? 55 : 31) && kBack % SLIDE == 0, "wide (160 slots, 129 taps), mid (96 slots, 65 taps) or far (120 slots, 65 taps)");
 	__device__ __forceinline__ void setup(uint32_t) {}
 	__device__ static __forceinline__ void place(const uint32_t (&f)[16], int c)
@@ -232,11 +244,14 @@
 	rotwin_demod<WinH<BLK, NA, MSL>, 32, OQPSK, 0>(L);
 }
 
+#ifndef ROT_VCONST
+#define ROT_VCONST 1
+#endif
 template <int FMT, int OQPSK, int KS, int COMPACT, int LUT>
 __global__ void __launch_bounds__(LUT ? MDEMOD_RW_LUT_BLOCK : MDEMOD_RW_BLOCK, 2) __attribute__((amdgpu_num_vgpr(ROTWIN_LIMIT / 2)))
 demod_kernel_rot(const DemodLaunch L)
 {
-	rotwin_demod<WinF<FMT, COMPACT, LUT ? MDEMOD_RW_LUT_BLOCK : MDEMOD_RW_BLOCK>, FMT, OQPSK, KS, LUT>(L);
+	rotwin_demod<WinF<FMT, COMPACT, LUT ? MDEMOD_RW_LUT_BLOCK : MDEMOD_RW_BLOCK, ROT_VCONST>, FMT, OQPSK, KS, LUT>(L);
 }
 
 template <int FMT, int OQPSK, int KS, int COMPACT = 0, int LUT = 0>
diff --git a/meteor_demod_amd/csrc/demod_kernel_rotp.hip b/meteor_demod_amd/csrc/demod_kernel_rotp.hip
--- a/meteor_demod_amd/csrc/demod_kernel_rotp.hip
+++ b/meteor_demod_amd/csrc/demod_kernel_rotp.hip
@@ -80,7 +80,7 @@
 struct WinP {
 	static constexpr int kTaps = GeoP<GEO>::kTaps, kBack = kTaps - 1, NW = GeoP<GEO>::NW, SLIDE = 16, AMAX = NW - kTaps,
 	                     MAXSL = GeoP<GEO>::MAXSL, DEPTH = GeoP<GEO>::DEPTH, BLOCK = GeoP<GEO>::BLOCK, NCH = NW / SLIDE, GD = FMT == 16 ? 16 : 8, REGSLOTS = 0, ROTN = NCH, RING = 32;
-	static constexpr bool GATHER = false;
+	static constexpr bool GATHER = false, SCALAR_SLIDE = false, VCONST = false;
 	__device__ __forceinline__ void setup(uint32_t) {}
 	static_assert(kBack % SLIDE == 0 && NW % SLIDE == 0, "history and window are whole chunks");
 
diff --git a/meteor_demod_amd/csrc/gen_rotwin_asm.py b/meteor_demod_amd/csrc/gen_rotwin_asm.py
--- a/meteor_demod_amd/csrc/gen_rotwin_asm.py
+++ b/meteor_demod_amd/csrc/gen_rotwin_asm.py
@@ -5,6 +5,7 @@
 WB = 96
 CB = None
 NCH = 10
+SLIDE = 8
 PAIRWAIT = int(os.environ.get("ROTWIN_PAIRWAIT", "1"))
 DC = int(os.environ.get("ROTWIN_DC", "1"))
 NBUF = 2 * (DC + 1) if PAIRWAIT else 4
@@ -38,6 +39,8 @@
     L = []
     if PK in (0, 2):
         L += ["v_mov_b32 %[ar], 0", "v_mov_b32 %[ai], 0"]
+    else:
+        L += ["v_mov_b64 %[acc], 0"]
     L += [load(h) for h in range(2 * DC if PAIRWAIT else D)]
     L += jump("fir", NCH)
     for r in range(NCH):
@@ -116,6 +119,10 @@
                     L += ["v_mov_b32 v%d, %%[f%d]" % (dst, 2 * s + comp)]
         L += ["s_branch .Lput_end_%="]
     L += [".Lput_end_%=:"]
+    L += ["s_add_i32 %%[base], %%[base], %d" % SLIDE,
+          "s_add_i32 %[rot], %[rot], 1",
+          "s_cmp_eq_u32 %%[rot], %d" % NCH,
+          "s_cselect_b32 %[rot], 0, %[rot]"]
     return L
 
 
@@ -187,6 +194,7 @@
     out.append("#define ROTWIN_CB %d" % CB)
     out.append("#define ROTWIN_LIMIT %d   /* first register the compiler may not use */" % (TB if PK in (2, 3) else CB))
     out.append("#define ROTWIN_NCH %d" % NCH)
+    out.append("#define ROTWIN_SLIDE %d" % SLIDE)
     out.append("#define ROTWIN_AB %d   /* first AccVGPR of the hybrid window's newer half */" % AB)
     out.append("#define ROTWIN_PK %d" % PK)
     out.append("#define ROTWIN_FIR_ASM \\\n" + q(fir()).replace("\n", " \\\n"))
diff --git a/meteor_demod_amd/csrc/rot_fir_bounds.h b/meteor_demod_amd/csrc/rot_fir_bounds.h
--- /dev/null
+++ b/meteor_demod_amd/csrc/rot_fir_bounds.h
@@ -0,0 +1,26 @@
+#ifndef MDEMOD_ROT_FIR_BOUNDS_H
+#define MDEMOD_ROT_FIR_BOUNDS_H
+
+#include <stdint.h>
+
+#if defined(__HIPCC__) || defined(__CUDACC__)
+#define ROT_FIR_HD __host__ __device__
+#else
+#define ROT_FIR_HD
+#endif
+
+struct RotFirQ { int q_lo, q_hi; };
+
+ROT_FIR_HD constexpr RotFirQ
+rot_fir_q(uint64_t ex, uint64_t m4, uint64_t m8, uint64_t m12)
+{
+	return RotFirQ{ m4 != ex ? 0 : (m8 != ex ? 1 : (m12 != ex ? 2 : 3)), m4 == 0 ? 0 : (m8 == 0 ? 1 : (m12 == 0 ? 2 : 3)) };
+}
+
+ROT_FIR_HD constexpr int
+rot_fir_flags(int q_lo, int q_hi)
+{
+	return ((1 << q_lo) - 1) | (((1 << (3 - q_hi)) - 1) << 3);
+}
+
+#endif
diff --git a/meteor_demod_amd/csrc/rotwin_asm.h b/meteor_demod_amd/csrc/rotwin_asm.h
--- a/meteor_demod_amd/csrc/rotwin_asm.h
+++ b/meteor_demod_amd/csrc/rotwin_asm.h
@@ -4,9 +4,11 @@
 #define ROTWIN_CB 80
 #define ROTWIN_LIMIT 80
 #define ROTWIN_NCH 10
+#define ROTWIN_SLIDE 8
 #define ROTWIN_AB 96
 #define ROTWIN_PK 1
 #define ROTWIN_FIR_ASM \
+	"v_mov_b64 %[acc], 0\n\t" \
 	"ds_read_b128 v[80:83], %[addr] offset:0\n\t" \
 	"ds_read_b128 v[84:87], %[addr] offset:16\n\t" \
 	"s_getpc_b64 vcc\n\t" \
@@ -2266,7 +2268,11 @@
 	"v_cvt_f32_i32_sdwa v254, sext(%[g7]) dst_sel:DWORD dst_unused:UNUSED_PAD src0_sel:WORD_0\n\t" \
 	"v_cvt_f32_i32_sdwa v255, sext(%[g7]) dst_sel:DWORD dst_unused:UNUSED_PAD src0_sel:WORD_1\n\t" \
 	"s_branch .Lput_end_%=\n\t" \
-	".Lput_end_%=:\n\t"
+	".Lput_end_%=:\n\t" \
+	"s_add_i32 %[base], %[base], 8\n\t" \
+	"s_add_i32 %[rot], %[rot], 1\n\t" \
+	"s_cmp_eq_u32 %[rot], 10\n\t" \
+	"s_cselect_b32 %[rot], 0, %[rot]\n\t"
 #define ROTWIN_PUT_U8_ASM \
 	"s_nop 1\n\t" \
 	"s_getpc_b64 vcc\n\t" \
@@ -2456,7 +2462,11 @@
 	"v_cvt_f32_i32_sdwa v254, sext(%[g3]) dst_sel:DWORD dst_unused:UNUSED_PAD src0_sel:BYTE_2\n\t" \
 	"v_cvt_f32_i32_sdwa v255, sext(%[g3]) dst_sel:DWORD dst_unused:UNUSED_PAD src0_sel:BYTE_3\n\t" \
 	"s_branch .Lput_end_%=\n\t" \
-	".Lput_end_%=:\n\t"
+	".Lput_end_%=:\n\t" \
+	"s_add_i32 %[base], %[base], 8\n\t" \
+	"s_add_i32 %[rot], %[rot], 1\n\t" \
+	"s_cmp_eq_u32 %[rot], 10\n\t" \
+	"s_cselect_b32 %[rot], 0, %[rot]\n\t"
 #define ROTWIN_PUT_F32_ASM \
 	"s_getpc_b64 vcc\n\t" \
 	".Lput_pc_%=:\n\t" \
@@ -2645,7 +2655,11 @@
 	"v_mov_b32 v254, %[f14]\n\t" \
 	"v_mov_b32 v255, %[f15]\n\t" \
 	"s_branch .Lput_end_%=\n\t" \
-	".Lput_end_%=:\n\t"
+	".Lput_end_%=:\n\t" \
+	"s_add_i32 %[base], %[base], 8\n\t" \
+	"s_add_i32 %[rot], %[rot], 1\n\t" \
+	"s_cmp_eq_u32 %[rot], 10\n\t" \
+	"s_cselect_b32 %[rot], 0, %[rot]\n\t"
 #define ROTWIN_FIR_ACC_ASM \
 	"ds_read_b128 v[80:83], %[addr] offset:0\n\t" \
 	"ds_read_b128 v[84:87], %[addr] offset:16\n\t" \
diff --git a/meteor_demod_amd/csrc/rotwin_body.h b/meteor_demod_amd/csrc/rotwin_body.h
--- a/meteor_demod_amd/csrc/rotwin_body.h
+++ b/meteor_demod_amd/csrc/rotwin_body.h
@@ -66,7 +66,7 @@
 struct RotClockConsts { int k_safe, steps_need, interp; float f_hi; uint32_t magic; float inv; const cj_sched *jump; rot_clktab_t tab; };
 template <int KS>
 __device__ __forceinline__ void
-rot_clock_fast(const RotClockConsts &K, float thr, int v_end, float &t_phase, float t_freq, int &isub, int &v_cur, int &bank, bool &fired, int jidx = -1)
+rot_clock_fast(const RotClockConsts &K, float thr, int v_end, int v_fast_end, float &t_phase, float t_freq, int &isub, int &v_cur, int &bank, bool &fired, int jidx = -1)
 {
 	int k_safe = KS ? KS : K.k_safe;
 	const int interp = K.interp;
@@ -75,7 +75,7 @@
 	const bool fast = (KS == 109 ? (t_phase > CJ109_P_LO && t_phase < CJ109_P_HI)
 	                   : jump    ? (t_phase > J.floor && t_phase < J.hi)
 	                             : (t_phase < thr - (float)k_safe * K.f_hi - 1e-3f))
-	                  && (v_cur + (jump ? J.need : K.steps_need) < v_end);
+	                  && (jump ? (v_cur + J.need < v_end) : (v_cur < v_fast_end));
 	if (fast) {
 		float p = t_phase;
 		if (KS == 109) k_safe = clock_jump_109(p, t_freq, thr, K.inv);
@@ -140,7 +140,10 @@
 	float *lut = ctab + L.ctab_floats;
 	enum { S_GAIN, S_BIAS_RE, S_BIAS_IM, S_PHASE, S_FREQ, S_ERR, S_FLAGS, S_TPREV, S_INPHASE, S_EVCALL, S_FIRSTLOCK, S_LASTV, S_COUNT };
 	static_assert(S_COUNT == MDEMOD_RW_STATE_SLOTS, "host LDS sizing");
-	float *sl = lut + 32 + (threadIdx.x >> 6) * (S_COUNT * 64) + (threadIdx.x & 63);
+	uint32_t sl_addr = (uint32_t)(uintptr_t)(__attribute__((address_space(3))) unsigned char *)lds
+	                   + 4u * (L.ctab_floats + 32u + (threadIdx.x >> 6) * (uint32_t)(S_COUNT * 64) + (threadIdx.x & 63u));
+	asm("" : "+v"(sl_addr));
+	float *sl = (float *)(__attribute__((address_space(3))) float *)(uintptr_t)sl_addr;
 	int *sli = reinterpret_cast<int *>(sl);
 	uint4 *stage = reinterpret_cast<uint4 *>(lut + 32 + (BLOCK / 64) * (S_COUNT * 64)) + threadIdx.x;
 	const uint32_t ctab_addr = (uint32_t)(uintptr_t)(__attribute__((address_space(3))) unsigned char *)lds;
@@ -226,6 +229,7 @@
 	int rot = 0;
 	int slot = 1;
 	int base = 0;
+	if constexpr (W::SCALAR_SLIDE) asm("s_mov_b32 %0, 0\n\ts_mov_b32 %1, 0" : "=s"(rot), "=s"(base));
 	int isub = 0, bank = interp - 1;
 	bool fired = false;
 	bool done = !valid || n == 0;
@@ -237,6 +241,9 @@
 	K.steps_need = ((KS == 109 ? CJ109_MAX_STEPS : C.step_safe) + 4 + C.interp - 1) / C.interp;
 	K.jump = C.jump;
 	K.tab = has_clktab ? (rot_clktab_t)clktab : (rot_clktab_t)0;
+	const int v_fast_end = v_end - K.steps_need;
+	float k_t_alpha = C.t_alpha, k_t_beta = C.t_beta, k_t_center = C.t_center, k_pll_alpha = C.pll_alpha, k_pll_beta = C.pll_beta;
+	if constexpr (W::VCONST) asm("" : "+v"(k_t_alpha), "+v"(k_t_beta), "+v"(k_t_center), "+v"(k_pll_alpha), "+v"(k_pll_beta));
 
 	int n_wave_max = n;
 	for (int o = 32; o > 0; o >>= 1) {
@@ -257,7 +264,7 @@
 		ROT_TICK(4);
 		if (!fired && !done) {
 			const float thr = OQPSK ? (float)dual_state * MD_PI_F : MD_TWO_PI_F;
-			rot_clock_fast<KS>(K, thr, v_end, t_phase, t_freq, isub, v_cur, bank, fired);
+			rot_clock_fast<KS>(K, thr, v_end, v_fast_end, t_phase, t_freq, isub, v_cur, bank, fired);
 			while (!fired && !done) {
 				if (isub == 0) {
 					if (v_cur + 1 >= v_end) { done = true; v_cur = V_DONE; break; }
@@ -285,9 +292,12 @@
 				RGran<FMT> g[GPS];
 #pragma unroll
 				for (int i = 0; i < GPS; i++) g[i] = stg[i];
-				win.put(g, __builtin_amdgcn_readfirstlane(rot));
-				rot = __builtin_amdgcn_readfirstlane((rot == ROTN - 1) ? 0 : rot + 1);
-				base = __builtin_amdgcn_readfirstlane(base + SLIDE);
+				if constexpr (W::SCALAR_SLIDE) win.slide(g, rot, base);
+				else {
+					win.put(g, __builtin_amdgcn_readfirstlane(rot));
+					rot = __builtin_amdgcn_readfirstlane((rot == ROTN - 1) ? 0 : rot + 1);
+					base = __builtin_amdgcn_readfirstlane(base + SLIDE);
+				}
 #pragma unroll
 				for (int i = 0; i + GPS < NST; i++) stg[i] = stg[i + GPS];
 				const int m_new = 4 * g_load;
@@ -309,7 +319,7 @@
 			fired = false;
 			cf32 y;
 			if constexpr (GATHER) win.fir_gather(ctab_addr, src, hist_in, v_cur, n, bank, C, y.re, y.im);
-			else win.fir(ctab_addr, a, bank, C, __builtin_amdgcn_readfirstlane(rot), y.re, y.im);
+			else win.fir(ctab_addr, a, bank, C, W::SCALAR_SLIDE ? rot : __builtin_amdgcn_readfirstlane(rot), y.re, y.im);
 			if (PRIO) __builtin_amdgcn_s_setprio(ROT_PRIO_LEVEL);
 			ROT_TICK(2);
 #ifdef ROT_EXP_TIMING
@@ -350,10 +360,10 @@
 				st_lastv(v_cur);
 				if (__builtin_expect(md_any(again), 0)) { if (again) sym_call--; }
 				float t_prev = ld_tprev();
-				md_timing_update(t_phase, t_freq, t_prev, C.t_alpha, C.t_beta, C.t_center, C.t_maxdev, out_im);
+				md_timing_update(t_phase, t_freq, t_prev, k_t_alpha, k_t_beta, k_t_center, C.t_maxdev, out_im);
 				st_tprev(t_prev);
 			}
-			rot_clock_fast<KS>(K, OQPSK ? (float)dual_state * MD_PI_F : MD_TWO_PI_F, v_end, t_phase, t_freq, isub, v_cur, bank, fired,
+			rot_clock_fast<KS>(K, OQPSK ? (float)dual_state * MD_PI_F : MD_TWO_PI_F, v_end, v_fast_end, t_phase, t_freq, isub, v_cur, bank, fired,
 			                   OQPSK ? (ROT_OQ_SYNC ? 2 - slot : -1) : 0);
 #ifdef ROT_EXP_TIMING
 			if (!fired) n_slide++;
@@ -361,7 +371,7 @@
 #endif
 			if (emit) {
 				uint32_t first = 0;
-				const uint32_t changed = md_pll_update_packed(pll, fl, lut, C.pll_alpha, C.pll_beta, C.pll_fmax, out_re, out_im, first);
+				const uint32_t changed = md_pll_update_packed(pll, fl, lut, k_pll_alpha, k_pll_beta, C.pll_fmax, out_re, out_im, first);
 				if (__builtin_expect(changed != 0, 0)) {
 					if (first) sli[S_FIRSTLOCK * 64] = (int)sym_call;
 					const int ev_call = sli[S_EVCALL * 64];
```
